# CliqueOfficial/zk-dcap-verifier

Measured on AMD Instinct MI355X. Metric: proofs/hour sgx_dcap_verifier k=19 (create_proof on the GPU: commitments, lookups, grand products, NTTs, evaluate_h, evaluations, SHPLONK, host transcript; witness synthesis excluded), higher is better.
Workload: dtype u32x8 (256-bit Montgomery integers)

## Files before the change

### zk-dcap-verifier_amd/csrc/capi.hip

```cpp
#include <string.h>
#include <new>
#include <system_error>
#include "quotient.h"

namespace zk {
int ntt_set_lds_attr();
int quotient_set_lds_attr();
int domain_lagrange_to_coeff(zk_ctx* ctx, void* d_a, uint32_t k);
int domain_coeff_to_lagrange(zk_ctx* ctx, void* d_a, uint32_t k);
int domain_lagrange_to_coeff_batch(zk_ctx* ctx, void* const* cols, size_t count, uint32_t k);
int domain_coeff_to_extended_batch(zk_ctx* ctx, const void* const* coeffs, void* const* outs, size_t count, uint32_t k, uint32_t ek);
int ntt_dev_batch(zk_ctx* ctx, void* const* h_cols, const void* const* h_srcs, size_t count, uint32_t log_n, const u256& omega, const NttFuse* fuse);
int domain_coeff_to_extended(zk_ctx* ctx, const void* d_coeff, uint32_t k, uint32_t ek, void* d_out);
int domain_extended_to_coeff(zk_ctx* ctx, void* d_a, uint32_t k, uint32_t ek);
int domain_divide_by_vanishing(zk_ctx* ctx, void* d_a, uint32_t k, uint32_t ek);
int fr_vec_op(zk_ctx* ctx, int op, const void* a, const void* b, void* out, size_t n, const u256* scalar);
int permutation_product(zk_ctx* ctx, const void* const* values, const void* const* sigmas, size_t count, uint32_t k, const void* beta, const void* gamma,
                        const void* delta_start, const void* z_init, const void* blinding, uint32_t bf, void* d_z, void* h_last_z);
int lookup_product(zk_ctx* ctx, const void* cin, const void* ctab, const void* pin, const void* ptab, uint32_t k, const void* beta, const void* gamma,
                   const void* blinding, uint32_t bf, void* d_z);
int permutation_product_circuits(zk_ctx* ctx, const void* const* values, const void* const* sigmas, size_t m, size_t n_circuits, uint32_t chunk_len, uint32_t k,
                                 const void* beta, const void* gamma, const void* blinding, uint32_t bf, void* const* d_zs);
int lookup_product_batch(zk_ctx* ctx, const void* const* cols4, size_t count, uint32_t k, const void* beta, const void* gamma, const void* blinding,
                         uint32_t bf, void* const* d_zs);
int eval_polynomial_batch(zk_ctx* ctx, const void* const* polys, size_t count, size_t n, const void* points, void* out);
int kate_division(zk_ctx* ctx, const void* d_a, size_t n, const void* b_host, void* d_q);
int fr_lincomb(zk_ctx* ctx, const void* const* polys, const void* scalars, size_t count, size_t n, void* d_out);
int pk_load(zk_ctx* ctx, uint64_t prog, const void* const* fixed, const void* const* sigma, const void* l0, const void* l_last, const void* l_active,
            int form, uint64_t* handle);
int pk_release(zk_ctx* ctx, uint64_t h);
void release_pks(zk_ctx* ctx);
int evaluate_h_host(zk_ctx* ctx, uint64_t pkh, const void* const* advice, const void* const* instance, const void* const* perm_products,
                    const void* const* lk_product, const void* const* lk_input, const void* const* lk_table, const void* challenges,
                    const void* beta, const void* gamma, const void* theta, const void* y, int finish, void* out);
int lookup_permute(zk_ctx* ctx, const void* d_input, const void* d_table, uint32_t k, uint32_t blinding_factors, const void* h_blind_input,
                   const void* h_blind_table, void* d_out_input, void* d_out_table);
int lookup_permute_batch(zk_ctx* ctx, const void* const* d_inputs, const void* const* d_tables, size_t count, uint32_t k, uint32_t blinding_factors,
                         const void* h_blind_inputs, const void* h_blind_tables, void* const* d_out_inputs, void* const* d_out_tables);
int g1_decompress(zk_ctx* ctx, const void* d_bytes, size_t n, uint32_t sign_bit, void* d_out_affine, uint32_t* n_bad_host);
int g1_compress(zk_ctx* ctx, const void* d_affine, size_t n, uint32_t sign_bit, void* d_bytes);
int g1_ntt(zk_ctx* ctx, const void* d_affine_in, uint32_t log_n, const void* omega_host, const void* scale_host, void* d_affine_out);
int quotient_program_load(zk_ctx* ctx, const void* blob, size_t len, uint64_t* prog);
int quotient_program_release(zk_ctx* ctx, uint64_t prog);
int quotient_program_info(zk_ctx* ctx, uint64_t prog, uint32_t* n_instr, uint32_t* n_slots, uint32_t* n_columns);
int quotient_program_kernels(zk_ctx* ctx, uint64_t prog, uint32_t* n_kernels);
int quotient_program_opmix(zk_ctx* ctx, uint64_t prog, uint32_t part, uint32_t counts[9]);
int mock_prover_verify(zk_ctx* ctx, const zk_mock_desc* d, zk_mock_failure* out, size_t cap, uint64_t counts[3], size_t* n_written, const void* challenges = nullptr,
                       uint32_t n_challenges = 0, bool phased = false);
int mock_prover_open(zk_ctx* ctx, const zk_mock_desc* d, uint64_t* mp);
int mock_prover_check(zk_ctx* ctx, uint64_t mp, const zk_mock_witness* w, zk_mock_failure* out, size_t cap, uint64_t counts[3], size_t* n_written);
int mock_prover_info(zk_ctx* ctx, uint64_t mp, zk_mock_info* info);
int mock_prover_close(zk_ctx* ctx, uint64_t mp);
int quotient_program_split(zk_ctx* ctx, uint64_t prog, uint32_t* low_cosets, uint32_t* n_instr_high, uint32_t* n_instr_low);
int domain_coeff_to_coset_batch(zk_ctx* ctx, const void* const* coeffs, void* const* outs, size_t count, uint32_t k, uint32_t ek, uint32_t coset);
int fr_interleave(zk_ctx* ctx, const void* const* h_cosets, size_t count, size_t n, void* d_out);
int domain_cosets_to_pieces(zk_ctx* ctx, void* const* h_numer, uint32_t q, uint32_t k, uint32_t ek, void* const* h_pieces);
}
using namespace zk;

int zk::abi_exception(zk_ctx* ctx, const char* fn) noexcept {
    int code = ZK_ERR_HIP;
    char msg[sizeof ctx->err];
    try { throw; }
    catch (const zk::AbiError& e) { code = e.code; snprintf(msg, sizeof msg, "%s: %s", fn, e.what ? e.what : "internal error"); }
    catch (const std::bad_alloc&) { code = ZK_ERR_LIMIT; snprintf(msg, sizeof msg, "%s: out of host memory (std::bad_alloc)", fn); }
    catch (const std::system_error& e) { snprintf(msg, sizeof msg, "%s: %s (std::system_error %d: no thread or lock to be had)", fn, e.what(), e.code().value()); }
    catch (const std::exception& e) { snprintf(msg, sizeof msg, "%s: unexpected C++ exception: %s", fn, e.what()); }
    catch (...) { snprintf(msg, sizeof msg, "%s: unexpected C++ exception", fn); }
    if (ctx) {
        try { std::lock_guard<std::mutex> lk(ctx->mu); memcpy(ctx->err, msg, sizeof msg); }
        catch (...) { memcpy(ctx->err, msg, sizeof msg); }
    }
    return code;
}

#ifdef ZK_FAULT_INJECT
#include <atomic>
namespace {
thread_local long g_fail_alloc_in = 0;
thread_local long g_alloc_count = 0;
std::atomic<long> g_fail_alloc_any{0};
thread_local int g_fail_thread = 0;
}
#if defined(__has_feature)
#if __has_feature(address_sanitizer) || __has_feature(thread_sanitizer)
#define ZK_NO_NEW_HOOK 1
#endif
#endif
#ifndef ZK_NO_NEW_HOOK
void* operator new(size_t n) {
    g_alloc_count++;
    if (g_fail_alloc_in > 0 && --g_fail_alloc_in == 0) throw std::bad_alloc();
    if (g_fail_alloc_any.load(std::memory_order_relaxed) > 0 && g_fail_alloc_any.fetch_sub(1) == 1) throw std::bad_alloc();
    void* p = malloc(n ? n : 1);
    if (!p) throw std::bad_alloc();
    return p;
}
void* operator new[](size_t n) { return operator new(n); }
void operator delete(void* p) noexcept { free(p); }
void operator delete[](void* p) noexcept { free(p); }
void operator delete(void* p, size_t) noexcept { free(p); }
void operator delete[](void* p, size_t) noexcept { free(p); }
#endif
void zk::fault_thread_tick() { if (g_fail_thread > 0 && --g_fail_thread == 0) throw std::system_error(std::make_error_code(std::errc::resource_unavailable_try_again), "std::thread"); }
extern "C" {
int zk_test_alloc_hook_present(void) {
#ifdef ZK_NO_NEW_HOOK
    return 0;
#else
    return 1;
#endif
}
void zk_test_fail_alloc(long nth) { g_fail_alloc_in = nth; g_alloc_count = 0; }
void zk_test_fail_alloc_any_thread(long nth) { g_fail_alloc_any.store(nth); }
long zk_test_alloc_count(void) { return g_alloc_count; }
void zk_test_fail_thread(int nth) { g_fail_thread = nth; }
#ifdef ZK_EMU
long zk_test_live_device_allocs(void) { return emu_live_device_allocs.load(); }
#endif
}
#endif

void zk_internal_plonk_ctx_destroyed(zk_ctx* ctx);
int zk_internal_fail(zk_ctx* ctx, int code, const char* msg) { return ctx ? ctx->fail(code, "%s", msg) : code; }
#define LOCK std::lock_guard<std::mutex> lk__(ctx->mu)
#define NEED_CTX if (!ctx) return ZK_ERR_ARG

extern "C" {

const char* zk_version(void) ZK_ABI_TRY {
#ifdef ZK_EMU
    return "zkmi355 0.1 (EMULATED kernels - test build, not the product)";
#else
    return "zkmi355 0.1 gfx950";
#endif
} ZK_ABI_CATCH_VALUE(nullptr, "zkmi355: internal error")

uint32_t zk_abi_version(void) ZK_ABI_TRY { return ZK_ABI_VERSION; } ZK_ABI_CATCH_VALUE(nullptr, 0u)
uint32_t zk_abi_struct_size(const char* name) ZK_ABI_TRY {
    if (!name) return 0;
    if (!strcmp(name, "zk_quotient_args")) return (uint32_t)sizeof(zk_quotient_args);
    if (!strcmp(name, "zk_plonk_pk_desc")) return (uint32_t)sizeof(zk_plonk_pk_desc);
    if (!strcmp(name, "zk_plonk_pk_host")) return (uint32_t)sizeof(zk_plonk_pk_host);
    if (!strcmp(name, "zk_mock_desc")) return (uint32_t)sizeof(zk_mock_desc);
    if (!strcmp(name, "zk_mock_failure")) return (uint32_t)sizeof(zk_mock_failure);
    if (!strcmp(name, "zk_plonk_phases")) return (uint32_t)sizeof(zk_plonk_phases);
    if (!strcmp(name, "zk_plonk_keygen_desc")) return (uint32_t)sizeof(zk_plonk_keygen_desc);
    if (!strcmp(name, "zk_mock_witness")) return (uint32_t)sizeof(zk_mock_witness);
    if (!strcmp(name, "zk_mock_info")) return (uint32_t)sizeof(zk_mock_info);
    return 0;
} ZK_ABI_CATCH_VALUE(nullptr, 0u)

int zk_ctx_create(int device_id, zk_ctx** out) ZK_ABI_TRY {
    if (!out) return ZK_ERR_ARG;
    *out = nullptr;
#ifndef ZK_EMU
    int ndev = 0;
    if (hipGetDeviceCount(&ndev) != hipSuccess || ndev <= 0 || device_id < 0 || device_id >= ndev) return ZK_ERR_NODEV;
    if (hipSetDevice(device_id) != hipSuccess) return ZK_ERR_NODEV;
#endif
    std::unique_ptr<zk_ctx> ctx(new zk_ctx());
    ctx->device = device_id;
    if (hipStreamCreateWithFlags(&ctx->stream, hipStreamNonBlocking) != hipSuccess) return ZK_ERR_HIP;
    msm_set_lds_attr();
    ntt_set_lds_attr();
    quotient_set_lds_attr();
    *out = ctx.release();
    return ZK_OK;
} ZK_ABI_CATCH(nullptr)

}
zk_ctx* zk_internal_helper_ctx(zk_ctx* ctx) {
    if (!ctx) return nullptr;
    zk_ctx* h;
    {
        LOCK;
        h = ctx->helper;
    }
    if (!h) {
        zk_ctx* made = nullptr;
        if (zk_ctx_create(ctx->device, &made) != ZK_OK) return nullptr;
#ifndef ZK_EMU
        {
            int lane_prio;
            { LOCK; lane_prio = ctx->tune.prover_lane_priority; }
            int least = 0, greatest = 0;
            hipStream_t s = nullptr;
            if (lane_prio && hipDeviceGetStreamPriorityRange(&least, &greatest) == hipSuccess && least != greatest &&
                hipStreamCreateWithPriority(&s, hipStreamNonBlocking, lane_prio == 1 ? least : greatest) == hipSuccess) {
                (void)hipStreamDestroy(made->stream);
                made->stream = s;
            }
        }
#endif
        {
            LOCK;
            if (!ctx->helper) { ctx->helper = made; made = nullptr; }
            h = ctx->helper;
        }
        if (made) zk_ctx_destroy(made);
    }
    zk::Tune t;
    bool timing;
    {
        LOCK;
        t = ctx->tune; timing = ctx->timing;
    }
    std::lock_guard<std::mutex> lk(h->mu);
    h->tune = t;
    h->timing = timing;
    return h;
}
static void release_workspaces(zk_ctx* ctx) {
    zk::DevBuf* bufs[] = {&ctx->ws_scalars, &ctx->ws_sorted, &ctx->ws_mid, &ctx->ws_small, &ctx->ws_sub0, &ctx->ws_sub1, &ctx->ws_cls0,
                          &ctx->ws_cls1, &ctx->ws_tmp, &ctx->ws_ntt, &ctx->ws_ntt_in, &ctx->ws_pts, &ctx->ws_runs, &ctx->ws_quot, &ctx->ws_quot_state};
    for (auto* b : bufs) b->release();
}
void zk_internal_trim_helper(zk_ctx* ctx) {
    if (!ctx) return;
    zk_ctx* h;
    { LOCK; h = ctx->helper; }
    if (!h) return;
    std::lock_guard<std::mutex> lk(h->mu);
    (void)hipSetDevice(h->device);
    (void)hipStreamSynchronize(h->stream);
    release_workspaces(h);
    release_twiddles(h);
}
extern "C" {
void zk_ctx_destroy(zk_ctx* ctx) ZK_ABI_TRY {
    if (!ctx) return;
    zk_ctx* helper;
    { LOCK; helper = ctx->helper; ctx->helper = nullptr; }
    if (helper) zk_ctx_destroy(helper);
    zk_internal_plonk_ctx_destroyed(ctx);
    (void)zk_plonk_trim(ctx);
    {
        LOCK;
        (void)hipSetDevice(ctx->device);
        (void)hipStreamSynchronize(ctx->stream);
        ctx->bases.clear();
        drop_pending_timers(ctx);
        release_twiddles(ctx);
        release_pks(ctx);
        release_mock_sessions(ctx);
        release_programs(ctx);
        release_gtab(ctx);
        release_workspaces(ctx);
        (void)hipStreamDestroy(ctx->stream);
    }
    delete ctx;
} ZK_ABI_CATCH_VOID(ctx)

const char* zk_last_error(zk_ctx* ctx) ZK_ABI_TRY { return ctx ? ctx->err : "null context"; } ZK_ABI_CATCH_VALUE(ctx, "zkmi355: internal error")

static int* tune_slot(zk_ctx* ctx, const char* key) {
    zk::Tune& t = ctx->tune;
    struct { const char* k; int* v; } tab[] = {
        {"msm_c", &t.msm_c}, {"msm_sort_wgs", &t.msm_sort_wgs}, {"msm_sort_threads", &t.msm_sort_threads}, {"msm_sort_batch_wgs", &t.msm_sort_batch_wgs}, {"msm_bsort_threads", &t.msm_bsort_threads}, {"msm_bsort_chunk", &t.msm_bsort_chunk}, {"msm_wide_bins_log", &t.msm_wide_bins_log}, {"msm_part_threads", &t.msm_part_threads}, {"msm_part_pairs", &t.msm_part_pairs}, {"msm_two_level_sort", &t.msm_two_level_sort},
        {"msm_target_threads", &t.msm_target_threads}, {"msm_min_chunk", &t.msm_min_chunk}, {"msm_max_chunk", &t.msm_max_chunk},
        {"msm_max_chunk_wide", &t.msm_max_chunk_wide}, {"msm_merge_fanin", &t.msm_merge_fanin}, {"msm_tree_fanin", &t.msm_tree_fanin}, {"msm_block", &t.msm_block}, {"msm_runs", &t.msm_runs}, {"prover_side_lane", &t.prover_side_lane}, {"prover_lane_priority", &t.prover_lane_priority},
        {"ntt_tile_log", &t.ntt_tile_log}, {"ntt_threads", &t.ntt_threads}, {"ntt_max_radix_log", &t.ntt_max_radix_log}, {"ntt_plan", &t.ntt_plan}, {"ntt_full_twiddle_max_log", &t.ntt_full_twiddle_max_log}, {"ntt_coset_table", &t.ntt_coset_table}, {"ntt_col_major", &t.ntt_col_major},
        {"vec_block", &t.vec_block}, {"quot_threads", &t.quot_threads},
        {"ntt_quarter_input", &t.ntt_quarter_input}, {"ntt_fuse_scale", &t.ntt_fuse_scale}, {"quot_piece_cosets", &t.quot_piece_cosets}, {"quot_factor_horner", &t.quot_factor_horner}, {"quot_degree_split", &t.quot_degree_split}, {"quot_group_factors", &t.quot_group_factors}, {"ntt_ws_limit_mb", &t.ntt_ws_limit_mb}, 
        {"quot_jit", &t.quot_jit}, {"quot_jit_group", &t.quot_jit_group}, {"quot_jit_waves", &t.quot_jit_waves}, {"quot_remat_ops", &t.quot_remat_ops}, {"quot_remat_distance", &t.quot_remat_distance}, {"keygen_wgs", &t.keygen_wgs}, {"mock_edge_wgs", &t.mock_edge_wgs}};
    for (auto& e : tab) if (!strcmp(e.k, key)) return e.v;
    return nullptr;
}
int zk_tune_set(zk_ctx* ctx, const char* key, int value) ZK_ABI_TRY {
    NEED_CTX; LOCK;
    int* s = key ? tune_slot(ctx, key) : nullptr;
    if (!s) return ctx->fail(ZK_ERR_ARG, "zk_tune_set: unknown key '%s'", key ? key : "(null)");
    if (value < 0) return ctx->fail(ZK_ERR_ARG, "zk_tune_set: negative value");
    *s = value;
    return ZK_OK;
} ZK_ABI_CATCH(ctx)
int zk_tune_get(zk_ctx* ctx, const char* key, int* value) ZK_ABI_TRY {
    NEED_CTX; LOCK;
    int* s = key ? tune_slot(ctx, key) : nullptr;
    if (!s || !value) return ctx->fail(ZK_ERR_ARG, "zk_tune_get: unknown key '%s'", key ? key : "(null)");
    *value = *s;
    return ZK_OK;
} ZK_ABI_CATCH(ctx)
int zk_timing_enable(zk_ctx* ctx, int on) ZK_ABI_TRY {
    NEED_CTX;
    zk_ctx* helper;
    { LOCK; helper = ctx->helper; }
    if (helper) (void)zk_timing_enable(helper, on);
    LOCK;
    resolve_pending_timers(ctx);
    if (on) ctx->last_ms.clear();
    ctx->timing = on != 0;
    return ZK_OK;
} ZK_ABI_CATCH(ctx)
double zk_timing_get(zk_ctx* ctx, const char* label) ZK_ABI_TRY {
    if (!ctx || !label) return -1.0;
    zk_ctx* helper;
    { LOCK; helper = ctx->helper; }
    const double side = helper ? zk_timing_get(helper, label) : -1.0;
    LOCK;
    resolve_pending_timers(ctx);
    auto it = ctx->last_ms.find(label);
    if (it == ctx->last_ms.end()) return side;
    return it->second + (side > 0 ? side : 0.0);
} ZK_ABI_CATCH_VALUE(ctx, -1.0)

#define ENTER NEED_CTX; LOCK; ZK_HIP(hipSetDevice(ctx->device))

int zk_dev_alloc(zk_ctx* ctx, size_t bytes, void** dptr) ZK_ABI_TRY { ENTER; if (!dptr) return ctx->fail(ZK_ERR_ARG, "null"); ZK_HIP(hipMalloc(dptr, bytes ? bytes : 32)); return ZK_OK; } ZK_ABI_CATCH(ctx)
int zk_dev_free(zk_ctx* ctx, void* dptr) ZK_ABI_TRY { ENTER; ZK_HIP(hipFree(dptr)); return ZK_OK; } ZK_ABI_CATCH(ctx)
int zk_dev_upload(zk_ctx* ctx, void* dptr, const void* host, size_t bytes) ZK_ABI_TRY {
    ENTER; if ((!dptr || !host) && bytes) return ctx->fail(ZK_ERR_ARG, "zk_dev_upload: null");
    ZK_HIP(hipMemcpyAsync(dptr, host, bytes, hipMemcpyHostToDevice, ctx->stream)); ZK_HIP(hipStreamSynchronize(ctx->stream)); return ZK_OK;
} ZK_ABI_CATCH(ctx)
int zk_dev_download(zk_ctx* ctx, void* host, const void* dptr, size_t bytes) ZK_ABI_TRY {
    ENTER; if ((!dptr || !host) && bytes) return ctx->fail(ZK_ERR_ARG, "zk_dev_download: null");
    ZK_HIP(hipMemcpyAsync(host, dptr, bytes, hipMemcpyDeviceToHost, ctx->stream)); ZK_HIP(hipStreamSynchronize(ctx->stream)); return ZK_OK;
} ZK_ABI_CATCH(ctx)
int zk_dev_copy(zk_ctx* ctx, void* dst, const void* src, size_t bytes) ZK_ABI_TRY {
    ENTER; if ((!dst || !src) && bytes) return ctx->fail(ZK_ERR_ARG, "zk_dev_copy: null");
    ZK_HIP(hipMemcpyAsync(dst, src, bytes, hipMemcpyDeviceToDevice, ctx->stream)); ZK_HIP(hipStreamSynchronize(ctx->stream)); return ZK_OK;
} ZK_ABI_CATCH(ctx)
int zk_dev_zero(zk_ctx* ctx, void* dptr, size_t bytes) ZK_ABI_TRY {
    ENTER; if (!dptr && bytes) return ctx->fail(ZK_ERR_ARG, "zk_dev_zero: null");
    ZK_HIP(hipMemsetAsync(dptr, 0, bytes, ctx->stream)); return ZK_OK;
} ZK_ABI_CATCH(ctx)
int zk_dev_sync(zk_ctx* ctx) ZK_ABI_TRY { ENTER; ZK_HIP(hipStreamSynchronize(ctx->stream)); return ZK_OK; } ZK_ABI_CATCH(ctx)
int zk_host_alloc(zk_ctx* ctx, size_t bytes, void** hptr) ZK_ABI_TRY {
    ENTER; if (!hptr) return ctx->fail(ZK_ERR_ARG, "zk_host_alloc: null");
    ZK_HIP(hipHostMalloc(hptr, bytes ? bytes : 32, 0)); return ZK_OK;
} ZK_ABI_CATCH(ctx)
int zk_host_free(zk_ctx* ctx, void* hptr) ZK_ABI_TRY { ENTER; ZK_HIP(hipHostFree(hptr)); return ZK_OK; } ZK_ABI_CATCH(ctx)
int zk_dev_upload_batch(zk_ctx* ctx, void* const* dptrs, const void* const* hosts, size_t count, size_t bytes_each) ZK_ABI_TRY {
    ENTER; if ((!dptrs || !hosts) && count) return ctx->fail(ZK_ERR_ARG, "zk_dev_upload_batch: null");
    for (size_t i = 0; i < count; i++) {
        if (!dptrs[i] || !hosts[i]) return ctx->fail(ZK_ERR_ARG, "zk_dev_upload_batch: null column %zu", i);
        ZK_HIP(hipMemcpyAsync(dptrs[i], hosts[i], bytes_each, hipMemcpyHostToDevice, ctx->stream));
    }
    ZK_HIP(hipStreamSynchronize(ctx->stream)); return ZK_OK;
} ZK_ABI_CATCH(ctx)

int zk_bases_register(zk_ctx* ctx, const void* p, size_t n, uint64_t* h) ZK_ABI_TRY { ENTER; return msm_register(ctx, p, n, false, h); } ZK_ABI_CATCH(ctx)
int zk_bases_register_dev(zk_ctx* ctx, const void* p, size_t n, uint64_t* h) ZK_ABI_TRY { ENTER; return msm_register(ctx, p, n, true, h); } ZK_ABI_CATCH(ctx)
int zk_bases_release(zk_ctx* ctx, uint64_t h) ZK_ABI_TRY { ENTER; return msm_release(ctx, h); } ZK_ABI_CATCH(ctx)
int zk_bases_enable_runs(zk_ctx* ctx, uint64_t h) ZK_ABI_TRY { ENTER; return msm_enable_runs(ctx, h); } ZK_ABI_CATCH(ctx)
int zk_bases_share(zk_ctx* ctx, zk_ctx* owner, uint64_t owner_handle, uint64_t* h) ZK_ABI_TRY {
    if (!ctx || !owner || !h) return ZK_ERR_ARG;
    zk::BaseTable bt;
    {
        std::lock_guard<std::mutex> lk(owner->mu);
        auto it = owner->bases.find(owner_handle);
        if (it == owner->bases.end()) return ZK_ERR_ARG;
        bt = it->second;
    }
    LOCK;
    if (owner->device != ctx->device) return ctx->fail(ZK_ERR_ARG, "zk_bases_share: the contexts are on different devices (%d, %d)", owner->device, ctx->device);
    return msm_share(ctx, bt, h);
} ZK_ABI_CATCH(ctx)
int zk_msm(zk_ctx* ctx, uint64_t b, const void* s, size_t n, void* out) ZK_ABI_TRY { ENTER; return msm_run(ctx, b, s, n, false, out, 0); } ZK_ABI_CATCH(ctx)
int zk_msm_dev(zk_ctx* ctx, uint64_t b, const void* s, size_t n, void* out) ZK_ABI_TRY { ENTER; return msm_run(ctx, b, s, n, true, out, 0); } ZK_ABI_CATCH(ctx)
int zk_msm_batch(zk_ctx* ctx, uint64_t b, const void* const* s, size_t count, size_t n, void* out) ZK_ABI_TRY { ENTER; return msm_run_batch(ctx, b, s, count, n, false, out, 0); } ZK_ABI_CATCH(ctx)
int zk_msm_batch_dev(zk_ctx* ctx, uint64_t b, const void* const* s, size_t count, size_t n, void* out) ZK_ABI_TRY { ENTER; return msm_run_batch(ctx, b, s, count, n, true, out, 0); } ZK_ABI_CATCH(ctx)
int zk_msm_partial_dev(zk_ctx* ctx, uint64_t b, const void* s, size_t n, void* out) ZK_ABI_TRY { ENTER; return msm_run(ctx, b, s, n, true, out, 1); } ZK_ABI_CATCH(ctx)
int zk_msm_batch_partial_dev(zk_ctx* ctx, uint64_t b, const void* const* s, size_t count, size_t n, void* out) ZK_ABI_TRY { ENTER; return msm_run_batch(ctx, b, s, count, n, true, out, 1); } ZK_ABI_CATCH(ctx)
int zk_g1_sum_xyzz_batch(const void* xyzz, size_t parts, size_t count, void* out) ZK_ABI_TRY {
    if (!xyzz || !out) return ZK_ERR_ARG;
    for (size_t c = 0; c < count; c++) {
        std::vector<unsigned char> col(parts * 128);
        for (size_t p = 0; p < parts; p++) memcpy(&col[p * 128], (const char*)xyzz + (p * count + c) * 128, 128);
        int rc = g1_sum_xyzz_host(col.data(), parts, (char*)out + c * 96);
        if (rc) return rc;
    }
    return ZK_OK;
} ZK_ABI_CATCH(nullptr)
int zk_g1_sum_xyzz(const void* xyzz, size_t count, void* out) ZK_ABI_TRY { if (!xyzz || !out) return ZK_ERR_ARG; return g1_sum_xyzz_host(xyzz, count, out); } ZK_ABI_CATCH(nullptr)
int zk_g1_fixed_base_mul_dev(zk_ctx* ctx, const void* s, size_t n, void* out) ZK_ABI_TRY { ENTER; return g1_fixed_base_mul(ctx, s, n, out); } ZK_ABI_CATCH(ctx)

int zk_g1_ntt_dev(zk_ctx* ctx, const void* in, uint32_t log_n, const void* omega, const void* scale, void* out) ZK_ABI_TRY { ENTER; return g1_ntt(ctx, in, log_n, omega, scale, out); } ZK_ABI_CATCH(ctx)

int zk_g1_decompress_dev(zk_ctx* ctx, const void* bytes_dev, size_t n, uint32_t sign_bit, void* out_affine_dev, uint32_t* n_invalid) ZK_ABI_TRY { ENTER; return g1_decompress(ctx, bytes_dev, n, sign_bit, out_affine_dev, n_invalid); } ZK_ABI_CATCH(ctx)
int zk_g1_compress_dev(zk_ctx* ctx, const void* affine_dev, size_t n, uint32_t sign_bit, void* bytes_dev) ZK_ABI_TRY { ENTER; return g1_compress(ctx, affine_dev, n, sign_bit, bytes_dev); } ZK_ABI_CATCH(ctx)

static int with_host_buffer(zk_ctx* ctx, void* host_in_out, size_t in_bytes, size_t buf_bytes, size_t out_bytes, void** dbuf) {
    ZK_HIP(ctx->ws_ntt_in.ensure(buf_bytes));
    *dbuf = ctx->ws_ntt_in.p;
    (void)out_bytes;
    ZK_HIP(hipMemcpyAsync(*dbuf, host_in_out, in_bytes, hipMemcpyHostToDevice, ctx->stream));
    return ZK_OK;
}
static int finish_host(zk_ctx* ctx, void* host, const void* dbuf, size_t bytes) {
    ZK_HIP(hipMemcpyAsync(host, dbuf, bytes, hipMemcpyDeviceToHost, ctx->stream));
    ZK_HIP(hipStreamSynchronize(ctx->stream));
    return ZK_OK;
}
static u256 load_host_fr(const void* p) { u256 o; memcpy(&o, p, 32); return o; }

int zk_ntt_dev(zk_ctx* ctx, void* a, uint32_t log_n, const void* omega) ZK_ABI_TRY {
    ENTER; if (!omega) return ctx->fail(ZK_ERR_ARG, "zk_ntt: null omega");
    int rc = ntt_dev(ctx, a, log_n, load_host_fr(omega), nullptr); if (rc) return rc;
    ZK_HIP(hipStreamSynchronize(ctx->stream)); return ZK_OK;
} ZK_ABI_CATCH(ctx)
int zk_ntt(zk_ctx* ctx, void* a, uint32_t log_n, const void* omega) ZK_ABI_TRY {
    ENTER; if (!omega || !a) return ctx->fail(ZK_ERR_ARG, "zk_ntt: null pointer");
    if (log_n > 27) return ctx->fail(ZK_ERR_LIMIT, "zk_ntt: log_n = %u > 27", log_n);
    void* d; size_t bytes = (size_t)32 << log_n;
    int rc = with_host_buffer(ctx, a, bytes, bytes, bytes, &d); if (rc) return rc;
    rc = ntt_dev(ctx, d, log_n, load_host_fr(omega), nullptr); if (rc) return rc;
    return finish_host(ctx, a, d, bytes);
} ZK_ABI_CATCH(ctx)
int zk_ntt_batch_dev(zk_ctx* ctx, void* const* cols, size_t count, uint32_t log_n, const void* omega) ZK_ABI_TRY {
    ENTER; if (!omega) return ctx->fail(ZK_ERR_ARG, "zk_ntt_batch_dev: null omega");
    int rc = ntt_dev_batch(ctx, cols, nullptr, count, log_n, load_host_fr(omega), nullptr); if (rc) return rc;
    ZK_HIP(hipStreamSynchronize(ctx->stream)); return ZK_OK;
} ZK_ABI_CATCH(ctx)
int zk_lagrange_to_coeff_batch_dev(zk_ctx* ctx, void* const* cols, size_t count, uint32_t k) ZK_ABI_TRY {
    ENTER; int rc = domain_lagrange_to_coeff_batch(ctx, cols, count, k); if (rc) return rc; ZK_HIP(hipStreamSynchronize(ctx->stream)); return ZK_OK;
} ZK_ABI_CATCH(ctx)
int zk_coeff_to_extended_batch_dev(zk_ctx* ctx, const void* const* coeffs, void* const* outs, size_t count, uint32_t k, uint32_t ek) ZK_ABI_TRY {
    ENTER; int rc = domain_coeff_to_extended_batch(ctx, coeffs, outs, count, k, ek); if (rc) return rc; ZK_HIP(hipStreamSynchronize(ctx->stream)); return ZK_OK;
} ZK_ABI_CATCH(ctx)
int zk_coeff_to_coset_batch_dev(zk_ctx* ctx, const void* const* coeffs, void* const* outs, size_t count, uint32_t k, uint32_t ek, uint32_t coset) ZK_ABI_TRY {
    ENTER; int rc = domain_coeff_to_coset_batch(ctx, coeffs, outs, count, k, ek, coset); if (rc) return rc; ZK_HIP(hipStreamSynchronize(ctx->stream)); return ZK_OK;
} ZK_ABI_CATCH(ctx)
int zk_fr_interleave_dev(zk_ctx* ctx, const void* const* cosets, size_t count, size_t n, void* out) ZK_ABI_TRY { ENTER; return fr_interleave(ctx, cosets, count, n, out); } ZK_ABI_CATCH(ctx)
int zk_cosets_to_pieces_dev(zk_ctx* ctx, void* const* numer, uint32_t pieces, uint32_t k, uint32_t ek, void* const* out) ZK_ABI_TRY { ENTER; return domain_cosets_to_pieces(ctx, numer, pieces, k, ek, out); } ZK_ABI_CATCH(ctx)
int zk_lagrange_to_coeff_dev(zk_ctx* ctx, void* a, uint32_t k) ZK_ABI_TRY { ENTER; int rc = domain_lagrange_to_coeff(ctx, a, k); if (rc) return rc; ZK_HIP(hipStreamSynchronize(ctx->stream)); return ZK_OK; } ZK_ABI_CATCH(ctx)
int zk_coeff_to_lagrange_dev(zk_ctx* ctx, void* a, uint32_t k) ZK_ABI_TRY { ENTER; int rc = domain_coeff_to_lagrange(ctx, a, k); if (rc) return rc; ZK_HIP(hipStreamSynchronize(ctx->stream)); return ZK_OK; } ZK_ABI_CATCH(ctx)
int zk_coeff_to_extended_dev(zk_ctx* ctx, const void* c, uint32_t k, uint32_t ek, void* out) ZK_ABI_TRY { ENTER; int rc = domain_coeff_to_extended(ctx, c, k, ek, out); if (rc) return rc; ZK_HIP(hipStreamSynchronize(ctx->stream)); return ZK_OK; } ZK_ABI_CATCH(ctx)
int zk_extended_to_coeff_dev(zk_ctx* ctx, void* a, uint32_t k, uint32_t ek) ZK_ABI_TRY { ENTER; int rc = domain_extended_to_coeff(ctx, a, k, ek); if (rc) return rc; ZK_HIP(hipStreamSynchronize(ctx->stream)); return ZK_OK; } ZK_ABI_CATCH(ctx)
int zk_divide_by_vanishing_poly_dev(zk_ctx* ctx, void* a, uint32_t k, uint32_t ek) ZK_ABI_TRY { ENTER; return domain_divide_by_vanishing(ctx, a, k, ek); } ZK_ABI_CATCH(ctx)

int zk_lagrange_to_coeff(zk_ctx* ctx, void* a, uint32_t k) ZK_ABI_TRY {
    ENTER; if (!a || k > 27) return ctx->fail(ZK_ERR_ARG, "zk_lagrange_to_coeff: bad argument");
    void* d; size_t bytes = (size_t)32 << k;
    int rc = with_host_buffer(ctx, a, bytes, bytes, bytes, &d); if (rc) return rc;
    rc = domain_lagrange_to_coeff(ctx, d, k); if (rc) return rc;
    return finish_host(ctx, a, d, bytes);
} ZK_ABI_CATCH(ctx)
int zk_coeff_to_extended(zk_ctx* ctx, const void* c, uint32_t k, uint32_t ek, void* out) ZK_ABI_TRY {
    ENTER; if (!c || !out || k > ek || ek > 27) return ctx->fail(ZK_ERR_ARG, "zk_coeff_to_extended: bad argument");
    size_t inb = (size_t)32 << k, outb = (size_t)32 << ek;
    ZK_HIP(ctx->ws_ntt_in.ensure(inb + outb));
    void* din = ctx->ws_ntt_in.p; void* dout = (char*)din + inb;
    ZK_HIP(hipMemcpyAsync(din, c, inb, hipMemcpyHostToDevice, ctx->stream));
    int rc = domain_coeff_to_extended(ctx, din, k, ek, dout); if (rc) return rc;
    return finish_host(ctx, out, dout, outb);
} ZK_ABI_CATCH(ctx)
int zk_extended_to_coeff(zk_ctx* ctx, void* a, uint32_t k, uint32_t ek) ZK_ABI_TRY {
    ENTER; if (!a || k > ek || ek > 27) return ctx->fail(ZK_ERR_ARG, "zk_extended_to_coeff: bad argument");
    void* d; size_t bytes = (size_t)32 << ek;
    int rc = with_host_buffer(ctx, a, bytes, bytes, bytes, &d); if (rc) return rc;
    rc = domain_extended_to_coeff(ctx, d, k, ek); if (rc) return rc;
    return finish_host(ctx, a, d, bytes);
} ZK_ABI_CATCH(ctx)

static int vec_sync(zk_ctx* ctx, int rc) { if (rc) return rc; ZK_HIP(hipStreamSynchronize(ctx->stream)); return ZK_OK; }
int zk_fr_mul_dev(zk_ctx* ctx, const void* a, const void* b, void* o, size_t n) ZK_ABI_TRY { ENTER; return vec_sync(ctx, fr_vec_op(ctx, 0, a, b, o, n, nullptr)); } ZK_ABI_CATCH(ctx)
int zk_fr_add_dev(zk_ctx* ctx, const void* a, const void* b, void* o, size_t n) ZK_ABI_TRY { ENTER; return vec_sync(ctx, fr_vec_op(ctx, 1, a, b, o, n, nullptr)); } ZK_ABI_CATCH(ctx)
int zk_fr_sub_dev(zk_ctx* ctx, const void* a, const void* b, void* o, size_t n) ZK_ABI_TRY { ENTER; return vec_sync(ctx, fr_vec_op(ctx, 2, a, b, o, n, nullptr)); } ZK_ABI_CATCH(ctx)
int zk_fr_scale_dev(zk_ctx* ctx, const void* a, const void* s, void* o, size_t n) ZK_ABI_TRY {
    ENTER; if (!s) return ctx->fail(ZK_ERR_ARG, "zk_fr_scale_dev: null scalar");
    u256 sc = load_host_fr(s); return vec_sync(ctx, fr_vec_op(ctx, 3, a, nullptr, o, n, &sc));
} ZK_ABI_CATCH(ctx)
int zk_fq_mul_dev(zk_ctx* ctx, const void* a, const void* b, void* o, size_t n) ZK_ABI_TRY { ENTER; return vec_sync(ctx, fr_vec_op(ctx, 4, a, b, o, n, nullptr)); } ZK_ABI_CATCH(ctx)

int zk_permutation_product_dev(zk_ctx* ctx, const void* const* values, const void* const* sigmas, size_t count, uint32_t k, const void* beta,
                               const void* gamma, const void* delta_start, const void* z_init, const void* blinding, uint32_t blinding_factors,
                               void* z_dev, void* last_z_out) ZK_ABI_TRY {
    ENTER; return permutation_product(ctx, values, sigmas, count, k, beta, gamma, delta_start, z_init, blinding, blinding_factors, z_dev, last_z_out);
} ZK_ABI_CATCH(ctx)
int zk_lookup_product_dev(zk_ctx* ctx, const void* cin, const void* ctab, const void* pin, const void* ptab, uint32_t k, const void* beta,
                          const void* gamma, const void* blinding, uint32_t blinding_factors, void* z_dev) ZK_ABI_TRY {
    ENTER; return lookup_product(ctx, cin, ctab, pin, ptab, k, beta, gamma, blinding, blinding_factors, z_dev);
} ZK_ABI_CATCH(ctx)

int zk_permutation_product_all_dev(zk_ctx* ctx, const void* const* values, const void* const* sigmas, size_t n_columns, uint32_t chunk_len, uint32_t k,
                                   const void* beta, const void* gamma, const void* blinding, uint32_t blinding_factors, void* const* z_devs) ZK_ABI_TRY {
    ENTER; return permutation_product_circuits(ctx, values, sigmas, n_columns, 1, chunk_len, k, beta, gamma, blinding, blinding_factors, z_devs);
} ZK_ABI_CATCH(ctx)
}
int zk_internal_permutation_products(zk_ctx* ctx, const void* const* values, const void* const* sigmas, size_t n_columns, size_t n_circuits, uint32_t chunk_len, uint32_t k,
                                     const void* beta, const void* gamma, const void* blinding, uint32_t blinding_factors, void* const* z_devs) {
    ENTER; return permutation_product_circuits(ctx, values, sigmas, n_columns, n_circuits, chunk_len, k, beta, gamma, blinding, blinding_factors, z_devs);
}
extern "C" {
int zk_lookup_product_batch_dev(zk_ctx* ctx, const void* const* cols4, size_t count, uint32_t k, const void* beta, const void* gamma, const void* blinding,
                                uint32_t blinding_factors, void* const* z_devs) ZK_ABI_TRY {
    ENTER; return lookup_product_batch(ctx, cols4, count, k, beta, gamma, blinding, blinding_factors, z_devs);
} ZK_ABI_CATCH(ctx)

int zk_lookup_permute_dev(zk_ctx* ctx, const void* input, const void* table, uint32_t k, uint32_t blinding_factors, const void* blind_input,
                          const void* blind_table, void* out_input, void* out_table) ZK_ABI_TRY {
    ENTER; return lookup_permute(ctx, input, table, k, blinding_factors, blind_input, blind_table, out_input, out_table);
} ZK_ABI_CATCH(ctx)

int zk_lookup_permute_batch_dev(zk_ctx* ctx, const void* const* inputs, const void* const* tables, size_t count, uint32_t k, uint32_t blinding_factors,
                                const void* blind_inputs, const void* blind_tables, void* const* out_inputs, void* const* out_tables) ZK_ABI_TRY {
    ENTER; return lookup_permute_batch(ctx, inputs, tables, count, k, blinding_factors, blind_inputs, blind_tables, out_inputs, out_tables);
} ZK_ABI_CATCH(ctx)

int zk_eval_polynomial_batch_dev(zk_ctx* ctx, const void* const* polys, size_t count, size_t n, const void* points, void* out) ZK_ABI_TRY {
    ENTER; return eval_polynomial_batch(ctx, polys, count, n, points, out);
} ZK_ABI_CATCH(ctx)
int zk_kate_division_dev(zk_ctx* ctx, const void* a_dev, size_t n, const void* b, void* q_dev) ZK_ABI_TRY { ENTER; return kate_division(ctx, a_dev, n, b, q_dev); } ZK_ABI_CATCH(ctx)
int zk_fr_lincomb_dev(zk_ctx* ctx, const void* const* polys_dev, const void* scalars, size_t count, size_t n, void* out_dev) ZK_ABI_TRY { ENTER; return fr_lincomb(ctx, polys_dev, scalars, count, n, out_dev); } ZK_ABI_CATCH(ctx)

int zk_quotient_program_load(zk_ctx* ctx, const void* blob, size_t len, uint64_t* prog) ZK_ABI_TRY { ENTER; return quotient_program_load(ctx, blob, len, prog); } ZK_ABI_CATCH(ctx)
int zk_quotient_program_info(zk_ctx* ctx, uint64_t prog, uint32_t* ni, uint32_t* ns, uint32_t* nc) ZK_ABI_TRY { ENTER; return quotient_program_info(ctx, prog, ni, ns, nc); } ZK_ABI_CATCH(ctx)
int zk_quotient_program_kernels(zk_ctx* ctx, uint64_t prog, uint32_t* n_kernels) ZK_ABI_TRY { ENTER; return quotient_program_kernels(ctx, prog, n_kernels); } ZK_ABI_CATCH(ctx)
int zk_quotient_program_opmix(zk_ctx* ctx, uint64_t prog, uint32_t counts[9]) ZK_ABI_TRY { ENTER; return quotient_program_opmix(ctx, prog, 0, counts); } ZK_ABI_CATCH(ctx)
int zk_quotient_program_part_opmix(zk_ctx* ctx, uint64_t prog, uint32_t part, uint32_t counts[9]) ZK_ABI_TRY { ENTER; return quotient_program_opmix(ctx, prog, part, counts); } ZK_ABI_CATCH(ctx)
int zk_quotient_program_release(zk_ctx* ctx, uint64_t prog) ZK_ABI_TRY { ENTER; return quotient_program_release(ctx, prog); } ZK_ABI_CATCH(ctx)
int zk_quotient_program_share(zk_ctx* ctx, zk_ctx* owner, uint64_t owner_prog, uint64_t* prog) ZK_ABI_TRY {
    if (!ctx || !owner || !prog) return ZK_ERR_ARG;
    return quotient_program_share(ctx, owner, owner_prog, prog);
} ZK_ABI_CATCH(ctx)
#define ARGS_SIZE(fn) do { if (!args) return ctx->fail(ZK_ERR_ARG, fn ": null args"); \
        if (args->struct_size != sizeof(zk_quotient_args)) return ctx->fail(ZK_ERR_ARG, fn ": zk_quotient_args.struct_size %u, expected %zu (ABI version %u)", args->struct_size, sizeof(zk_quotient_args), ZK_ABI_VERSION); } while (0)
int zk_mock_prover_verify(zk_ctx* ctx, const zk_mock_desc* desc, zk_mock_failure* out, size_t cap, uint64_t counts[3], size_t* n_written) ZK_ABI_TRY {
    ENTER; return mock_prover_verify(ctx, desc, out, cap, counts, n_written);
} ZK_ABI_CATCH(ctx)
int zk_mock_prover_verify_phased(zk_ctx* ctx, const zk_mock_desc* desc, const void* challenges, uint32_t n_challenges, zk_mock_failure* out, size_t cap,
                                 uint64_t counts[3], size_t* n_written) ZK_ABI_TRY {
    ENTER;
    if (n_challenges && !challenges) return ctx->fail(ZK_ERR_ARG, "zk_mock_prover_verify_phased: %u challenges and a null array", n_challenges);
    if (n_challenges > ZK_MAX_CHALLENGES) return ctx->fail(ZK_ERR_LIMIT, "zk_mock_prover_verify_phased: %u challenges, the quotient interpreter's constant bank is sized for %u", n_challenges, ZK_MAX_CHALLENGES);
    return mock_prover_verify(ctx, desc, out, cap, counts, n_written, challenges, n_challenges, true);
} ZK_ABI_CATCH(ctx)
int zk_mock_prover_open(zk_ctx* ctx, const zk_mock_desc* desc, uint64_t* mp) ZK_ABI_TRY { ENTER; return mock_prover_open(ctx, desc, mp); } ZK_ABI_CATCH(ctx)
int zk_mock_prover_check(zk_ctx* ctx, uint64_t mp, const zk_mock_witness* w, zk_mock_failure* out, size_t cap, uint64_t counts[3], size_t* n_written) ZK_ABI_TRY {
    ENTER; return mock_prover_check(ctx, mp, w, out, cap, counts, n_written);
} ZK_ABI_CATCH(ctx)
int zk_mock_prover_info(zk_ctx* ctx, uint64_t mp, zk_mock_info* info) ZK_ABI_TRY { ENTER; return mock_prover_info(ctx, mp, info); } ZK_ABI_CATCH(ctx)
int zk_mock_prover_close(zk_ctx* ctx, uint64_t mp) ZK_ABI_TRY { ENTER; return mock_prover_close(ctx, mp); } ZK_ABI_CATCH(ctx)
int zk_quotient_run_dev(zk_ctx* ctx, uint64_t prog, const zk_quotient_args* args) ZK_ABI_TRY { ENTER; ARGS_SIZE("zk_quotient_run_dev"); return quotient_run(ctx, prog, args, QuotRoute{}); } ZK_ABI_CATCH(ctx)
int zk_quotient_run_coset_dev(zk_ctx* ctx, uint64_t prog, const zk_quotient_args* args, uint32_t coset) ZK_ABI_TRY {
    ENTER;
    ARGS_SIZE("zk_quotient_run_coset_dev");
    if (coset >= (1u << 16)) return ctx->fail(ZK_ERR_ARG, "zk_quotient_run_coset_dev: coset %u out of range", coset);
    QuotRoute r;
    r.coset = (int)coset;
    return quotient_run(ctx, prog, args, r);
} ZK_ABI_CATCH(ctx)
int zk_quotient_run_coset_rows_dev(zk_ctx* ctx, uint64_t prog, const zk_quotient_args* args, uint32_t coset, uint64_t row_lo, uint64_t row_count) ZK_ABI_TRY {
    ENTER;
    ARGS_SIZE("zk_quotient_run_coset_rows_dev");
    if (coset >= (1u << 16)) return ctx->fail(ZK_ERR_ARG, "zk_quotient_run_coset_rows_dev: coset %u out of range", coset);
    if (!row_count) return ctx->fail(ZK_ERR_ARG, "zk_quotient_run_coset_rows_dev: row_count = 0");
    QuotRoute r;
    r.coset = (int)coset; r.row_lo = row_lo; r.row_count = row_count;
    return quotient_run(ctx, prog, args, r);
} ZK_ABI_CATCH(ctx)
int zk_quotient_program_split(zk_ctx* ctx, uint64_t prog, uint32_t* low_cosets, uint32_t* n_instr_high, uint32_t* n_instr_low) ZK_ABI_TRY { ENTER; return quotient_program_split(ctx, prog, low_cosets, n_instr_high, n_instr_low); } ZK_ABI_CATCH(ctx)
int zk_quotient_run_high_dev(zk_ctx* ctx, uint64_t prog, const zk_quotient_args* args) ZK_ABI_TRY {
    ENTER; ARGS_SIZE("zk_quotient_run_high_dev");
    QuotRoute r;
    r.part = 1;
    return quotient_run(ctx, prog, args, r);
} ZK_ABI_CATCH(ctx)
int zk_quotient_run_low_dev(zk_ctx* ctx, uint64_t prog, const zk_quotient_args* args, uint32_t low_cosets) ZK_ABI_TRY {
    ENTER; ARGS_SIZE("zk_quotient_run_low_dev");
    if (!low_cosets) return ctx->fail(ZK_ERR_ARG, "zk_quotient_run_low_dev: low_cosets = 0");
    QuotRoute r;
    r.part = 2; r.low_cosets = low_cosets;
    return quotient_run(ctx, prog, args, r);
} ZK_ABI_CATCH(ctx)
int zk_quotient_run_coset_part_dev(zk_ctx* ctx, uint64_t prog, const zk_quotient_args* args, uint32_t coset, uint32_t part) ZK_ABI_TRY {
    ENTER; ARGS_SIZE("zk_quotient_run_coset_part_dev");
    if (coset >= (1u << 16) || part < 1 || part > 2) return ctx->fail(ZK_ERR_ARG, "zk_quotient_run_coset_part_dev: coset %u / part %u out of range", coset, part);
    QuotRoute r;
    r.coset = (int)coset; r.part = (int)part;
    return quotient_run(ctx, prog, args, r);
} ZK_ABI_CATCH(ctx)
int zk_quotient_run_acc_dev(zk_ctx* ctx, uint64_t prog, const zk_quotient_args* args, uint32_t coset, uint32_t part) ZK_ABI_TRY {
    ENTER; ARGS_SIZE("zk_quotient_run_acc_dev");
    if ((coset != UINT32_MAX && coset >= (1u << 16)) || part > 2) return ctx->fail(ZK_ERR_ARG, "zk_quotient_run_acc_dev: coset %u / part %u out of range", coset, part);
    QuotRoute r;
    r.coset = coset == UINT32_MAX ? -1 : (int)coset; r.part = (int)part; r.accumulate = true;
    if (coset == UINT32_MAX && part == 2) {
        int rc = quotient_program_split(ctx, prog, &r.low_cosets, nullptr, nullptr);
        if (rc) return rc;
        if (!r.low_cosets) return ctx->fail(ZK_ERR_ARG, "zk_quotient_run_acc_dev: program %llu has no degree split (zk_quotient_program_split)", (unsigned long long)prog);
    }
    return quotient_run(ctx, prog, args, r);
} ZK_ABI_CATCH(ctx)

int zk_pk_load(zk_ctx* ctx, uint64_t prog, const void* const* fixed, const void* const* sigma, const void* l0, const void* l_last, const void* l_active,
               int form, uint64_t* pk) ZK_ABI_TRY { ENTER; return pk_load(ctx, prog, fixed, sigma, l0, l_last, l_active, form, pk); } ZK_ABI_CATCH(ctx)
int zk_pk_release(zk_ctx* ctx, uint64_t pk) ZK_ABI_TRY { ENTER; return pk_release(ctx, pk); } ZK_ABI_CATCH(ctx)
int zk_evaluate_h(zk_ctx* ctx, uint64_t pk, const void* const* advice, const void* const* instance, const void* const* perm_products,
                  const void* const* lookup_product, const void* const* lookup_input, const void* const* lookup_table, const void* challenges,
                  const void* beta, const void* gamma, const void* theta, const void* y, int finish, void* out) ZK_ABI_TRY {
    ENTER; return evaluate_h_host(ctx, pk, advice, instance, perm_products, lookup_product, lookup_input, lookup_table, challenges, beta, gamma, theta, y, finish, out);
} ZK_ABI_CATCH(ctx)

}
```

### zk-dcap-verifier_amd/csrc/ctx.h

```cpp
#pragma once
#include <stdarg.h>
#include <string.h>
#include <stdio.h>
#include <list>
#include <map>
#include <memory>
#include <mutex>
#include <string>
#include <vector>
#include "ec.cuh"
#include "../../include/zkmi355.h"
#include "abi_guard.h"

namespace zk {

struct Tune {
    int msm_c = 0;
    int msm_sort_wgs = 256;
    int msm_sort_threads = 1024;
    int msm_bsort_threads = 1024;
    int msm_bsort_chunk = 8192;
    int msm_part_threads = 1024, msm_part_pairs = 16384;
    int msm_wide_bins_log = 9;
    int msm_two_level_sort = 0;
    int msm_sort_batch_wgs = 2048;
    int msm_target_threads = 1 << 19;
    int msm_min_chunk = 16;
    int msm_max_chunk = 48;
    int msm_max_chunk_wide = 128;
    int msm_merge_fanin = 8;
    int msm_tree_fanin = 2;
    int msm_block = 128;
    int prover_lane_priority = 1;
    int prover_side_lane = 1;
    int msm_runs = 1;
    int ntt_tile_log = 10;
    int ntt_threads = 256;
    int ntt_max_radix_log = 8;
    int ntt_plan = 0;
    int ntt_col_major = 1;
    int ntt_coset_table = 1;
    int ntt_full_twiddle_max_log = 24;
    int ntt_ws_limit_mb = 24576;
    int ntt_fuse_scale = 1;
    int ntt_quarter_input = 1;
    int vec_block = 256;
    int quot_threads = 128;
    int quot_piece_cosets = 1;
    int quot_degree_split = 1;
    int quot_group_factors = 1;
    int quot_factor_horner = 1;
    int quot_remat_ops = 4;
    int quot_remat_distance = 24;
    int quot_jit = 0;
    int quot_jit_waves = 0;
    int keygen_wgs = 2048;
    int mock_edge_wgs = 2048;
    int quot_jit_group = 200;
};

struct DevBuf {
    void* p = nullptr;
    size_t cap = 0;
    hipError_t ensure(size_t bytes) {
        if (bytes <= cap) return hipSuccess;
        if (p) (void)hipFree(p);
        p = nullptr; cap = 0;
        size_t want = bytes + bytes / 8 + 4096;
        hipError_t e = hipMalloc(&p, want);
        if (e == hipSuccess) cap = want;
        return e;
    }
    void release() { if (p) (void)hipFree(p); p = nullptr; cap = 0; }
};

struct DevTmp {
    void* p = nullptr;
    DevTmp() = default;
    DevTmp(const DevTmp&) = delete;
    DevTmp& operator=(const DevTmp&) = delete;
    ~DevTmp() { if (p) (void)hipFree(p); }
    void* release() { void* q = p; p = nullptr; return q; }
    void reset() { if (p) (void)hipFree(p); p = nullptr; }
};

struct TableMem {
    void* p = nullptr;
    int device = 0;
    ~TableMem() { if (p) { (void)hipSetDevice(device); (void)hipFree(p); } }
};
struct BaseTable {
    void* d_table = nullptr;
    size_t n = 0;
    int c = 0, W = 0;
    std::shared_ptr<TableMem> mem;
    void* d_runs_table = nullptr;
    std::shared_ptr<TableMem> runs_mem;
};

struct TwiddleSet {
    uint32_t log_n = 0;
    u256 omega;
    void* d_lo = nullptr;
    void* d_hi = nullptr;
    uint32_t lo_bits = 0;
    void* d_stage[3] = {nullptr, nullptr, nullptr};
    void* d_stage_sh[3] = {nullptr, nullptr, nullptr};
    void* d_stage29[3] = {nullptr, nullptr, nullptr};
    void* d_full[3] = {nullptr, nullptr, nullptr};
    uint32_t radix_log[3] = {0, 0, 0};
    int passes = 0;
    bool scale_fused = false;
    u256 fused_scale;
    uint64_t stamp = 0;
};

struct QuotProgram;
struct MockSession;

}

struct zk_ctx {
    int device = 0;
    std::mutex mu;
    char err[640] = {0};
    hipStream_t stream = nullptr;
    zk::Tune tune;
    uint64_t next_handle = 1;
    std::map<uint64_t, zk::BaseTable> bases;
    std::list<zk::TwiddleSet> twiddles;
    uint64_t twiddle_clock = 0;
    std::map<uint64_t, void*> coset_tables;
    std::map<uint64_t, std::shared_ptr<zk::QuotProgram>> programs;
    std::map<uint64_t, std::shared_ptr<zk::MockSession>> mock_sessions;
    std::map<uint64_t, std::vector<uint32_t>> lookup_tie_hint;
    zk::DevBuf ws_scalars, ws_sorted, ws_mid, ws_small, ws_sub0, ws_sub1, ws_cls0, ws_cls1, ws_tmp, ws_ntt, ws_ntt_in, ws_pts, ws_runs, ws_quot, ws_quot_state;
    bool timing = false;
    std::map<std::string, double> last_ms;
    struct PendingTimer { const char* label; hipEvent_t a, b; };
    std::vector<PendingTimer> pending_timers;
    zk_ctx* helper = nullptr;

    int fail(int code, const char* fmt, ...) {
        char buf[sizeof err];
        va_list ap;
        va_start(ap, fmt);
        vsnprintf(buf, sizeof buf, fmt, ap);
        va_end(ap);
        memcpy(err, buf, sizeof err);
        return code;
    }
};

#define ZK_HIP(call)                                                                          \
    do {                                                                                      \
        hipError_t e__ = (call);                                                              \
        if (e__ != hipSuccess)                                                                \
            return ctx->fail(ZK_ERR_HIP, "%s failed: %s (%s:%d)", #call, hipGetErrorString(e__), __FILE__, __LINE__); \
    } while (0)
#define ZK_CHECK_LAUNCH() ZK_HIP(hipGetLastError())

namespace zk {
inline void resolve_pending_timers(zk_ctx* ctx);
struct EvTimer {
    zk_ctx* ctx; const char* label; hipEvent_t a = nullptr, b = nullptr; bool on;
    EvTimer(zk_ctx* c, const char* l) : ctx(c), label(l), on(c->timing) {
        if (on) { (void)hipEventCreate(&a); (void)hipEventCreate(&b); (void)hipEventRecord(a, ctx->stream); }
    }
    void stop() { if (on) (void)hipEventRecord(b, ctx->stream); }
    void resolve() {
        if (!on) return;
        (void)hipEventSynchronize(b);
        float ms = 0; (void)hipEventElapsedTime(&ms, a, b);
        on = false;
        (void)hipEventDestroy(a); (void)hipEventDestroy(b);
        ctx->last_ms[label] += ms; ctx->last_ms[std::string(label) + "#n"] += 1.0;
    }
    void defer() {
        if (!on) return;
        if (ctx->pending_timers.size() >= 4096) resolve_pending_timers(ctx);
        ctx->pending_timers.push_back({label, a, b});
        on = false;
    }
    ~EvTimer() { if (on) { (void)hipEventDestroy(a); (void)hipEventDestroy(b); } }
    EvTimer(const EvTimer&) = delete;
    EvTimer& operator=(const EvTimer&) = delete;
};
inline void resolve_pending_timers(zk_ctx* ctx) {
    std::vector<zk_ctx::PendingTimer> list;
    list.swap(ctx->pending_timers);
    struct Drop { std::vector<zk_ctx::PendingTimer>& l; ~Drop() { for (auto& t : l) { (void)hipEventDestroy(t.a); (void)hipEventDestroy(t.b); } } } drop{list};
    for (auto& t : list) {
        (void)hipEventSynchronize(t.b);
        float ms = 0; (void)hipEventElapsedTime(&ms, t.a, t.b);
        ctx->last_ms[t.label] += ms; ctx->last_ms[std::string(t.label) + "#n"] += 1.0;
    }
}
inline void drop_pending_timers(zk_ctx* ctx) {
    for (auto& t : ctx->pending_timers) { (void)hipEventDestroy(t.a); (void)hipEventDestroy(t.b); }
    ctx->pending_timers.clear();
}

int msm_register(zk_ctx* ctx, const void* pts, size_t n, bool on_device, uint64_t* handle);
int msm_release(zk_ctx* ctx, uint64_t handle);
int msm_share(zk_ctx* dst, const BaseTable& bt, uint64_t* handle);
int msm_enable_runs(zk_ctx* ctx, uint64_t handle);
int msm_run(zk_ctx* ctx, uint64_t handle, const void* scalars, size_t n, bool on_device, void* out, int partial);
int msm_run_batch(zk_ctx* ctx, uint64_t handle, const void* const* scalars, size_t nb, size_t n, bool on_device, void* out, int partial);
int g1_sum_xyzz_host(const void* xyzz, size_t count, void* out_jac);
int g1_fixed_base_mul(zk_ctx* ctx, const void* d_scalars, size_t n, void* d_out_affine);
void release_gtab(zk_ctx* ctx);
int msm_set_lds_attr();
struct NttFuse {
    const void* src = nullptr;
    uint32_t n_valid = 0;
    int pre_zeta = 0;
    int post_scale = 0;
    u256 scale;
    int post_zeta_inv = 0;
    const void* cs_lo = nullptr; const void* cs_hi = nullptr; uint32_t cs_lo_bits = 0, cs_stride = 0, cs_log = 0;
    const void* pre_full = nullptr;
};
int ntt_dev(zk_ctx* ctx, void* d_a, uint32_t log_n, const u256& omega, const NttFuse* fuse);
void release_twiddles(zk_ctx* ctx);
void release_programs(zk_ctx* ctx);
void release_mock_sessions(zk_ctx* ctx);
int quotient_program_share(zk_ctx* ctx, zk_ctx* owner, uint64_t owner_prog, uint64_t* prog);
}
```

### zk-dcap-verifier_amd/csrc/lookupperm.hip

```cpp
#include "ctx.h"
#include <vector>

namespace zk {

constexpr uint32_t FS_T = 256, FS_E = 16, FS_TILE = FS_T * FS_E, FS_PAD = 258;

ZK_HD uint32_t fs_digit(uint2 k, uint32_t pass) { return ((pass < 4 ? k.x : k.y) >> (8 * (pass & 3))) & 255u; }

constexpr uint32_t XS_T = 256, XS_E = 8, XS_TILE = XS_T * XS_E;

ZK_HD int lp_cmp(const u256& a, const u256& b) {
    for (int i = 7; i >= 0; i--) {
        if (a.v[i] < b.v[i]) return -1;
        if (a.v[i] > b.v[i]) return 1;
    }
    return 0;
}
static uint32_t lp_scan_threads(uint32_t m) {
    uint32_t t = 64;
    while (t < 1024 && t * 8 < m) t <<= 1;
    return t;
}

struct LpbArgs {
    const void* const* cols;
    void* const* outs;
    const void* const* scols;
    const uint32_t* tabcol;
    uint32_t u, n, nb, S, C, nwg, nxs;
    void* canon; uint2* key_a; uint2* key_b; uint32_t* idx_a; uint32_t* idx_b;
    uint32_t* flags; uint32_t* ranks; uint32_t* leftover; uint32_t* ghist; uint32_t* xsums; uint32_t* scal;
    uint32_t* cscal;
    const uint32_t* shifts;
    const void* blind;
};
ZK_KERNEL void lpb_canon_kernel(LpbArgs a) {
    __shared__ uint32_t lor[8];
    const uint32_t s = blockIdx.y, i = blockIdx.x * blockDim.x + threadIdx.x;
    if (threadIdx.x < 8) lor[threadIdx.x] = 0;
    __syncthreads();
    if (i < a.u) {
        const u256 c = Fr::from_mont(load_u256(a.scols[s], i));
        store_u256(a.canon, (size_t)s * a.u + i, c);
#pragma unroll
        for (int w = 0; w < 8; w++) if (c.v[w] & ~lor[w]) atomicOr(&lor[w], c.v[w]);
    }
    __syncthreads();
    if (threadIdx.x < 8 && lor[threadIdx.x]) atomicOr(&a.cscal[s * 16 + threadIdx.x], lor[threadIdx.x]);
}
ZK_KERNEL void lpb_keys_kernel(LpbArgs a) {
    const uint32_t s = blockIdx.y, i = blockIdx.x * blockDim.x + threadIdx.x;
    if (i >= a.u) return;
    const uint32_t shift = a.shifts[s];
    const uint32_t* w = reinterpret_cast<const uint32_t*>(a.canon) + ((size_t)s * a.u + i) * 8;
    const uint32_t ws = shift >> 5, bs = shift & 31;
    uint32_t x[3];
#pragma unroll
    for (int j = 0; j < 3; j++) x[j] = ws + j < 8 ? w[ws + j] : 0u;
    uint2 k;
    k.x = bs ? (x[0] >> bs) | (x[1] << (32 - bs)) : x[0];
    k.y = bs ? (x[1] >> bs) | (x[2] << (32 - bs)) : x[1];
    a.key_a[(size_t)s * a.u + i] = k;
    a.idx_a[(size_t)s * a.u + i] = i;
}
ZK_KERNEL void lpb_hist_kernel(const uint2* keys, uint32_t u, uint32_t pass, uint32_t* ghist, uint32_t nwg) {
    __shared__ uint32_t lh[256];
    const uint32_t s = blockIdx.y, tid = threadIdx.x, base = blockIdx.x * FS_TILE;
    keys += (size_t)s * u;
    lh[tid] = 0;
    __syncthreads();
    for (uint32_t e = 0; e < FS_E; e++) {
        const uint32_t i = base + e * FS_T + tid;
        bool live = i < u;
        const uint32_t d = live ? fs_digit(keys[i], pass) : 0u;
#ifndef ZK_EMU
#pragma unroll
        for (int round = 0; round < 2; round++) {
            if (live) {
                const uint32_t lead = (uint32_t)__builtin_amdgcn_readfirstlane((int)d);
                const bool same = d == lead;
                const unsigned long long m = __ballot(same);
                if (same) {
                    if ((__lane_id() & 63u) == (uint32_t)__builtin_ctzll(m)) atomicAdd(&lh[lead], (uint32_t)__builtin_popcountll(m));
                    live = false;
                }
            }
        }
#endif
        if (live) atomicAdd(&lh[d], 1u);
    }
    __syncthreads();
    ghist[((size_t)s * nwg + blockIdx.x) * 256 + tid] = lh[tid];
}
ZK_KERNEL void lpb_offsets_kernel(uint32_t* ghist, uint32_t nwg) {
    __shared__ uint32_t scan[256];
    const uint32_t s = blockIdx.x, tid = threadIdx.x;
    uint32_t* h = ghist + (size_t)s * nwg * 256;
    uint32_t total = 0;
    for (uint32_t w = 0; w < nwg; w++) total += h[(size_t)w * 256 + tid];
    scan[tid] = total;
    __syncthreads();
    for (uint32_t d = 1; d < 256; d <<= 1) {
        const uint32_t add = tid >= d ? scan[tid - d] : 0;
        __syncthreads();
        scan[tid] += add;
        __syncthreads();
    }
    uint32_t run = scan[tid] - total;
    for (uint32_t w = 0; w < nwg; w++) {
        const uint32_t c = h[(size_t)w * 256 + tid];
        h[(size_t)w * 256 + tid] = run;
        run += c;
    }
}
ZK_KERNEL void lpb_scatter_kernel(const uint2* keys_in, const uint32_t* idx_in, uint2* keys_out, uint32_t* idx_out, uint32_t u, uint32_t pass,
                                  const uint32_t* gbase_all, uint32_t nwg) {
    __shared__ __attribute__((aligned(16))) uint16_t cnt[FS_T * FS_PAD];
    __shared__ uint32_t gbase[256];
    const uint32_t s = blockIdx.y, tid = threadIdx.x, wg = blockIdx.x, base = wg * FS_TILE;
    keys_in += (size_t)s * u; idx_in += (size_t)s * u; keys_out += (size_t)s * u; idx_out += (size_t)s * u;
    {
        uint4* c4 = reinterpret_cast<uint4*>(cnt);
        constexpr uint32_t n4 = FS_T * FS_PAD * 2 / 16;
        for (uint32_t q = tid; q < n4; q += FS_T) c4[q] = make_uint4(0, 0, 0, 0);
    }
    gbase[tid] = gbase_all[((size_t)s * nwg + wg) * 256 + tid];
    __syncthreads();
    uint2 k[FS_E];
    uint32_t v[FS_E];
    uint16_t rl[FS_E];
    const uint32_t lo = base + tid * FS_E;
#pragma unroll
    for (uint32_t e = 0; e < FS_E; e++) {
        const uint32_t i = lo + e;
        if (i < u) {
            k[e] = keys_in[i]; v[e] = idx_in[i];
            rl[e] = cnt[tid * FS_PAD + fs_digit(k[e], pass)]++;
        }
    }
    __syncthreads();
    {
        uint32_t run = 0;
        for (uint32_t t = 0; t < FS_T; t++) {
            const uint32_t c = cnt[t * FS_PAD + tid];
            cnt[t * FS_PAD + tid] = (uint16_t)run;
            run += c;
        }
    }
    __syncthreads();
#pragma unroll
    for (uint32_t e = 0; e < FS_E; e++) {
        const uint32_t i = lo + e;
        if (i < u) {
            const uint32_t d = fs_digit(k[e], pass);
            const uint32_t pos = gbase[d] + cnt[tid * FS_PAD + d] + rl[e];
            keys_out[pos] = k[e];
            idx_out[pos] = v[e];
        }
    }
}
ZK_KERNEL void lpb_check_kernel(LpbArgs a, const uint32_t* idx_sorted) {
    const uint32_t s = blockIdx.y, i = blockIdx.x * blockDim.x + threadIdx.x;
    if (i == 0 || i >= a.u || a.shifts[s] == 0) return;
    const uint32_t* canon = reinterpret_cast<const uint32_t*>(a.canon) + (size_t)s * a.u * 8;
    const uint32_t* idx = idx_sorted + (size_t)s * a.u;
    const uint32_t* x = canon + (size_t)idx[i - 1] * 8;
    const uint32_t* y = canon + (size_t)idx[i] * 8;
    for (int w = 7; w >= 0; w--) {
        if (x[w] < y[w]) return;
        if (x[w] > y[w]) { atomicAdd(&a.cscal[s * 16 + 8], 1u); return; }
    }
}
ZK_KERNEL void lpb_tiemask_kernel(LpbArgs a, const uint32_t* idx_sorted) {
    __shared__ uint32_t lor[8];
    const uint32_t s = blockIdx.y, i = blockIdx.x * blockDim.x + threadIdx.x;
    if (a.cscal[s * 16 + 8] == 0) return;
    if (threadIdx.x < 8) lor[threadIdx.x] = 0;
    __syncthreads();
    if (i > 0 && i < a.u) {
        const uint32_t shift = a.shifts[s];
        const uint32_t* canon = reinterpret_cast<const uint32_t*>(a.canon) + (size_t)s * a.u * 8;
        const uint32_t* idx = idx_sorted + (size_t)s * a.u;
        const uint32_t* x = canon + (size_t)idx[i - 1] * 8;
        const uint32_t* y = canon + (size_t)idx[i] * 8;
        uint32_t d[8], above = 0;
#pragma unroll
        for (int w = 0; w < 8; w++) {
            d[w] = x[w] ^ y[w];
            const uint32_t lo_bit = (uint32_t)w * 32;
            uint32_t in_window = lo_bit + 32 <= shift ? 0u : (lo_bit >= shift ? 0xffffffffu : (0xffffffffu << (shift - lo_bit)));
            above |= d[w] & in_window;
        }
        if (above == 0) {
#pragma unroll
            for (int w = 0; w < 8; w++) if (d[w] & ~lor[w]) atomicOr(&lor[w], d[w]);
        }
    }
    __syncthreads();
    if (threadIdx.x < 8 && lor[threadIdx.x]) atomicOr(&a.cscal[s * 16 + threadIdx.x], lor[threadIdx.x]);
}
ZK_KERNEL void lpb_rekey_kernel(LpbArgs a, const uint32_t* fcols, const uint32_t* fshift, const uint32_t* idx_in, uint2* key_out, uint32_t* idx_out) {
    const uint32_t f = blockIdx.y, i = blockIdx.x * blockDim.x + threadIdx.x;
    if (i >= a.u) return;
    const uint32_t c = fcols[f], shift = fshift[f];
    const uint32_t r = idx_in ? idx_in[(size_t)f * a.u + i] : i;
    const uint32_t* w = reinterpret_cast<const uint32_t*>(a.canon) + ((size_t)c * a.u + r) * 8;
    const uint32_t ws = shift >> 5, bs = shift & 31;
    uint32_t x[3];
#pragma unroll
    for (int j = 0; j < 3; j++) x[j] = ws + j < 8 ? w[ws + j] : 0u;
    uint2 k;
    k.x = bs ? (x[0] >> bs) | (x[1] << (32 - bs)) : x[0];
    k.y = bs ? (x[1] >> bs) | (x[2] << (32 - bs)) : x[1];
    key_out[(size_t)f * a.u + i] = k;
    idx_out[(size_t)f * a.u + i] = r;
}
ZK_KERNEL void lpb_mark_kernel(LpbArgs a, const uint32_t* idx_sorted) {
    const uint32_t l = blockIdx.y, i = blockIdx.x * blockDim.x + threadIdx.x, u = a.u;
    if (i >= u) return;
    const uint32_t tc = a.tabcol[l];
    const void* in_canon = (const char*)a.canon + (size_t)l * u * 32;
    const void* tab_canon = (const char*)a.canon + (size_t)tc * u * 32;
    const uint32_t* in_idx = idx_sorted + (size_t)l * u;
    const uint32_t* tab_idx = idx_sorted + (size_t)tc * u;
    uint32_t* repeated = a.flags + (size_t)(2 * l) * u;
    uint32_t* unconsumed = a.flags + (size_t)(2 * l + 1) * u;
    const u256 v = load_u256(in_canon, in_idx[i]);
    const bool first = i == 0 || lp_cmp(v, load_u256(in_canon, in_idx[i - 1])) != 0;
    repeated[i] = first ? 0u : 1u;
    if (!first) return;
    uint32_t lo = 0, hi = u;
    while (lo < hi) {
        const uint32_t mid = (lo + hi) >> 1;
        if (lp_cmp(load_u256(tab_canon, tab_idx[mid]), v) < 0) lo = mid + 1; else hi = mid;
    }
    if (lo >= u || lp_cmp(load_u256(tab_canon, tab_idx[lo]), v) != 0) { atomicAdd(&a.scal[l * 16 + 1], 1u); return; }
    unconsumed[lo] = 0;
}
ZK_KERNEL void lpb_fill_unconsumed_kernel(LpbArgs a) {
    const uint32_t l = blockIdx.y, i = blockIdx.x * blockDim.x + threadIdx.x;
    if (i < a.u) a.flags[(size_t)(2 * l + 1) * a.u + i] = 1u;
}
ZK_KERNEL void lpb_tile_sum_kernel(LpbArgs a) {
    __shared__ uint32_t part[XS_T];
    const uint32_t s = blockIdx.y, tid = threadIdx.x, base = blockIdx.x * XS_TILE;
    const uint32_t* v = a.ranks + (size_t)s * a.u;
    uint32_t sum = 0;
    for (uint32_t e = 0; e < XS_E; e++) { const uint32_t i = base + e * XS_T + tid; if (i < a.u) sum += v[i]; }
    part[tid] = sum;
    __syncthreads();
    for (uint32_t d = XS_T >> 1; d > 0; d >>= 1) { if (tid < d) part[tid] += part[tid + d]; __syncthreads(); }
    if (tid == 0) a.xsums[(size_t)s * a.nxs + blockIdx.x] = part[0];
}
ZK_KERNEL void lpb_sum_scan_kernel(LpbArgs a) {
    __shared__ uint32_t part[1024];
    const uint32_t s = blockIdx.x, T = blockDim.x, tid = threadIdx.x, m = a.nxs - 1;
    uint32_t* v = a.xsums + (size_t)s * a.nxs;
    const uint32_t per = (m + T - 1) / T;
    const uint32_t lo = tid * per < m ? tid * per : m, hi = lo + per < m ? lo + per : m;
    uint32_t sum = 0;
    for (uint32_t i = lo; i < hi; i++) sum += v[i];
    part[tid] = sum;
    __syncthreads();
    for (uint32_t d = 1; d < T; d <<= 1) {
        const uint32_t add = tid >= d ? part[tid - d] : 0;
        __syncthreads();
        part[tid] += add;
        __syncthreads();
    }
    uint32_t run = part[tid] - sum;
    for (uint32_t i = lo; i < hi; i++) { const uint32_t x = v[i]; v[i] = run; run += x; }
    if (tid == T - 1) a.scal[(s >> 1) * 16 + 2 + (s & 1)] = part[T - 1];
}
ZK_KERNEL void lpb_apply_kernel(LpbArgs a) {
    __shared__ uint32_t part[XS_T];
    const uint32_t s = blockIdx.y, tid = threadIdx.x, lo = blockIdx.x * XS_TILE + tid * XS_E, m = a.u;
    uint32_t* v = a.ranks + (size_t)s * a.u;
    uint32_t x[XS_E], sum = 0;
#pragma unroll
    for (uint32_t e = 0; e < XS_E; e++) { x[e] = lo + e < m ? v[lo + e] : 0u; sum += x[e]; }
    part[tid] = sum;
    __syncthreads();
    for (uint32_t d = 1; d < XS_T; d <<= 1) {
        const uint32_t add = tid >= d ? part[tid - d] : 0;
        __syncthreads();
        part[tid] += add;
        __syncthreads();
    }
    uint32_t run = a.xsums[(size_t)s * a.nxs + blockIdx.x] + part[tid] - sum;
#pragma unroll
    for (uint32_t e = 0; e < XS_E; e++) { if (lo + e < m) v[lo + e] = run; run += x[e]; }
}
ZK_KERNEL void lpb_compact_kernel(LpbArgs a) {
    const uint32_t l = blockIdx.y, t = blockIdx.x * blockDim.x + threadIdx.x;
    if (t < a.u && a.flags[(size_t)(2 * l + 1) * a.u + t]) a.leftover[(size_t)l * a.u + a.ranks[(size_t)(2 * l + 1) * a.u + t]] = t;
}
ZK_KERNEL void lpb_assemble_kernel(LpbArgs a, const uint32_t* idx_sorted) {
    const uint32_t l = blockIdx.y, i = blockIdx.x * blockDim.x + threadIdx.x, u = a.u;
    if (i >= a.n) return;
    void* out_in = a.outs[2 * l];
    void* out_tab = a.outs[2 * l + 1];
    if (i >= u) {
        store_u256(out_in, i, load_u256(a.blind, (size_t)(2 * l) * a.nb + (i - u)));
        store_u256(out_tab, i, load_u256(a.blind, (size_t)(2 * l + 1) * a.nb + (i - u)));
        return;
    }
    const uint32_t* in_idx = idx_sorted + (size_t)l * u;
    const uint32_t* tab_idx = idx_sorted + (size_t)a.tabcol[l] * u;
    const u256 v = load_u256(a.cols[2 * l], in_idx[i]);
    store_u256(out_in, i, v);
    if (!a.flags[(size_t)(2 * l) * u + i]) store_u256(out_tab, i, v);
    else {
        const uint32_t n_rep = a.scal[l * 16 + 2];
        store_u256(out_tab, i, load_u256(a.cols[2 * l + 1], tab_idx[a.leftover[(size_t)l * u + (n_rep - 1 - a.ranks[(size_t)(2 * l) * u + i])]]));
    }
}

int lookup_permute_batch(zk_ctx* ctx, const void* const* d_inputs, const void* const* d_tables, size_t count, uint32_t k, uint32_t blinding_factors,
                         const void* h_blind_inputs, const void* h_blind_tables, void* const* d_out_inputs, void* const* d_out_tables) {
    if (count == 0) return ZK_OK;
    if (!d_inputs || !d_tables || !d_out_inputs || !d_out_tables || !h_blind_inputs || !h_blind_tables)
        return ctx->fail(ZK_ERR_ARG, "zk_lookup_permute_batch_dev: null argument");
    if (k < 1 || k > 26 || count > 4096) return ctx->fail(ZK_ERR_ARG, "zk_lookup_permute_batch_dev: k = %u / count = %zu out of range", k, count);
    const uint32_t n = 1u << k, nb = blinding_factors + 1;
    if (nb >= n) return ctx->fail(ZK_ERR_ARG, "zk_lookup_permute_batch_dev: blinding_factors too large");
    for (size_t l = 0; l < count; l++)
        if (!d_inputs[l] || !d_tables[l] || !d_out_inputs[l] || !d_out_tables[l]) return ctx->fail(ZK_ERR_ARG, "zk_lookup_permute_batch_dev: null column %zu", l);
    const uint32_t u = n - nb, S = 2 * (uint32_t)count;
    std::vector<const void*> scols(d_inputs, d_inputs + count);
    std::vector<uint32_t> tabcol(count);
    for (size_t l = 0; l < count; l++) {
        size_t c = count;
        while (c < scols.size() && scols[c] != d_tables[l]) c++;
        if (c == scols.size()) scols.push_back(d_tables[l]);
        tabcol[l] = (uint32_t)c;
    }
    const uint32_t C = (uint32_t)scols.size();
    const uint32_t nwg = (u + FS_TILE - 1) / FS_TILE, nxs = (u + XS_TILE - 1) / XS_TILE + 1;
    size_t off = 0;
    auto take = [&](size_t bytes) { size_t o = off; off += (bytes + 255) & ~(size_t)255; return o; };
    const size_t o_canon = take((size_t)C * u * 32), o_blind = take((size_t)S * nb * 32), o_ka = take((size_t)C * u * 8), o_kb = take((size_t)C * u * 8),
                 o_ia = take((size_t)C * u * 4), o_ib = take((size_t)C * u * 4), o_fl = take((size_t)S * u * 4), o_rk = take((size_t)S * u * 4),
                 o_lo = take((size_t)count * u * 4), o_gh = take((size_t)C * nwg * 256 * 4), o_xs = take((size_t)S * nxs * 4), o_sc = take((size_t)count * 64),
                 o_cs = take((size_t)C * 64), o_sh = take((size_t)C * 4), o_tc = take((size_t)count * 4), o_cp = take((size_t)S * sizeof(void*)),
                 o_op = take((size_t)S * sizeof(void*)), o_sp = take((size_t)C * sizeof(void*));
    ZK_HIP(ctx->ws_tmp.ensure(off + 256));
    char* base = (char*)ctx->ws_tmp.p;
    hipStream_t st = ctx->stream;
    std::vector<const void*> cols(S);
    std::vector<void*> outs(S);
    std::vector<unsigned char> blind((size_t)S * nb * 32);
    for (size_t l = 0; l < count; l++) {
        cols[2 * l] = d_inputs[l]; cols[2 * l + 1] = d_tables[l];
        outs[2 * l] = d_out_inputs[l]; outs[2 * l + 1] = d_out_tables[l];
        memcpy(&blind[(2 * l) * (size_t)nb * 32], (const char*)h_blind_inputs + l * (size_t)nb * 32, (size_t)nb * 32);
        memcpy(&blind[(2 * l + 1) * (size_t)nb * 32], (const char*)h_blind_tables + l * (size_t)nb * 32, (size_t)nb * 32);
    }
    ZK_HIP(hipMemcpyAsync(base + o_cp, cols.data(), S * sizeof(void*), hipMemcpyHostToDevice, st));
    ZK_HIP(hipMemcpyAsync(base + o_op, outs.data(), S * sizeof(void*), hipMemcpyHostToDevice, st));
    ZK_HIP(hipMemcpyAsync(base + o_sp, scols.data(), C * sizeof(void*), hipMemcpyHostToDevice, st));
    ZK_HIP(hipMemcpyAsync(base + o_tc, tabcol.data(), count * 4, hipMemcpyHostToDevice, st));
    ZK_HIP(hipMemcpyAsync(base + o_blind, blind.data(), blind.size(), hipMemcpyHostToDevice, st));
    ZK_HIP(hipMemsetAsync(base + o_sc, 0, count * 64, st));
    ZK_HIP(hipMemsetAsync(base + o_cs, 0, (size_t)C * 64, st));
    LpbArgs a;
    memset(&a, 0, sizeof a);
    a.cols = (const void* const*)(base + o_cp); a.outs = (void* const*)(base + o_op); a.scols = (const void* const*)(base + o_sp);
    a.tabcol = (const uint32_t*)(base + o_tc);
    a.u = u; a.n = n; a.nb = nb; a.S = S; a.C = C; a.nwg = nwg; a.nxs = nxs;
    a.canon = base + o_canon; a.key_a = (uint2*)(base + o_ka); a.key_b = (uint2*)(base + o_kb); a.idx_a = (uint32_t*)(base + o_ia); a.idx_b = (uint32_t*)(base + o_ib);
    a.flags = (uint32_t*)(base + o_fl); a.ranks = (uint32_t*)(base + o_rk); a.leftover = (uint32_t*)(base + o_lo); a.ghist = (uint32_t*)(base + o_gh);
    a.xsums = (uint32_t*)(base + o_xs); a.scal = (uint32_t*)(base + o_sc); a.cscal = (uint32_t*)(base + o_cs); a.shifts = (const uint32_t*)(base + o_sh);
    a.blind = base + o_blind;
    const int blk = ctx->tune.vec_block;
    const uint32_t g = (u + blk - 1) / blk;
    ZK_LAUNCH(lpb_canon_kernel, dim3(g, C), blk, 0, st, a);
    ZK_CHECK_LAUNCH();
    std::vector<uint32_t> sc((size_t)count * 16), csc((size_t)C * 16);
    ZK_HIP(hipMemcpyAsync(csc.data(), a.cscal, (size_t)C * 64, hipMemcpyDeviceToHost, st));
    ZK_HIP(hipStreamSynchronize(st));
    std::vector<uint32_t> shifts(C);
    uint32_t max_bits = 1;
    bool any_shift = false;
    for (uint32_t c = 0; c < C; c++) {
        const uint32_t* om = &csc[(size_t)c * 16];
        uint32_t nbits = 1;
        for (int wd = 7; wd >= 0; wd--)
            if (om[wd]) { uint32_t top = 31; while (!((om[wd] >> top) & 1)) top--; nbits = (uint32_t)wd * 32 + top + 1; break; }
        shifts[c] = nbits > 64 ? nbits - 64 : 0;
        any_shift |= shifts[c] != 0;
        max_bits = std::max(max_bits, std::min(nbits, 64u));
    }
    ZK_HIP(hipMemcpyAsync(base + o_sh, shifts.data(), (size_t)C * 4, hipMemcpyHostToDevice, st));
    uint32_t* sorted = a.idx_a;
    const bool use_order_check = any_shift;

    auto compact_sort = [&](const std::vector<uint32_t>& fcols, const std::vector<std::vector<uint32_t>>& stage_shift, const std::vector<uint32_t>& stage_bits) -> int {
        const uint32_t Fn = (uint32_t)fcols.size();
        if (!Fn) return ZK_OK;
        const size_t per = (size_t)Fn * u;
        size_t o2 = 0;
        auto take2 = [&](size_t bytes) { size_t o = o2; o2 += (bytes + 255) & ~(size_t)255; return o; };
        const size_t q_ka = take2(per * 8), q_kb = take2(per * 8), q_ia = take2(per * 4), q_ib = take2(per * 4), q_gh = take2((size_t)Fn * nwg * 256 * 4),
                     q_fc = take2((size_t)Fn * 4), q_fs = take2((size_t)Fn * 4 * stage_shift.size());
        ZK_HIP(ctx->ws_mid.ensure(o2 + 256));
        char* b2 = (char*)ctx->ws_mid.p;
        uint2 *rk_in = (uint2*)(b2 + q_ka), *rk_out = (uint2*)(b2 + q_kb);
        uint32_t *ri_in = (uint32_t*)(b2 + q_ia), *ri_out = (uint32_t*)(b2 + q_ib), *rgh = (uint32_t*)(b2 + q_gh);
        ZK_HIP(hipMemcpyAsync(b2 + q_fc, fcols.data(), (size_t)Fn * 4, hipMemcpyHostToDevice, st));
        for (size_t t = 0; t < stage_shift.size(); t++)
            ZK_HIP(hipMemcpyAsync(b2 + q_fs + t * Fn * 4, stage_shift[t].data(), (size_t)Fn * 4, hipMemcpyHostToDevice, st));
        const uint32_t* order = nullptr;
        for (size_t t = 0; t < stage_shift.size(); t++) {
            ZK_LAUNCH(lpb_rekey_kernel, dim3(g, Fn), blk, 0, st, a, (const uint32_t*)(b2 + q_fc), (const uint32_t*)(b2 + q_fs + t * Fn * 4), order, rk_in, ri_in);
            ZK_CHECK_LAUNCH();
            const uint32_t ps = (stage_bits[t] + 7) / 8;
            for (uint32_t p = 0; p < ps; p++) {
                ZK_LAUNCH(lpb_hist_kernel, dim3(nwg, Fn), FS_T, 0, st, (const uint2*)rk_in, u, p, rgh, nwg);
                ZK_CHECK_LAUNCH();
                ZK_LAUNCH(lpb_offsets_kernel, Fn, 256, 0, st, rgh, nwg);
                ZK_CHECK_LAUNCH();
                ZK_LAUNCH(lpb_scatter_kernel, dim3(nwg, Fn), FS_T, 0, st, (const uint2*)rk_in, (const uint32_t*)ri_in, rk_out, ri_out, u, p, (const uint32_t*)rgh, nwg);
                ZK_CHECK_LAUNCH();
                std::swap(rk_in, rk_out);
                std::swap(ri_in, ri_out);
            }
            std::swap(rk_in, rk_out);
            std::swap(ri_in, ri_out);
            order = ri_out;
        }
        for (uint32_t f = 0; f < Fn; f++)
            ZK_HIP(hipMemcpyAsync(sorted + (size_t)fcols[f] * u, order + (size_t)f * u, (size_t)u * 4, hipMemcpyDeviceToDevice, st));
        return ZK_OK;
    };
    auto low_stages = [&](const std::vector<uint32_t>& fcols, const std::vector<uint32_t>& lo_bit, const std::vector<uint32_t>& hi_bit,
                          std::vector<std::vector<uint32_t>>& stage_shift, std::vector<uint32_t>& stage_bits) {
        const uint32_t Fn = (uint32_t)fcols.size();
        uint32_t n_low = 0;
        for (uint32_t f = 0; f < Fn; f++) if (lo_bit[f] < 256) n_low = std::max(n_low, (hi_bit[f] - lo_bit[f]) / 64 + 1);
        for (uint32_t t = 0; t < n_low; t++) {
            std::vector<uint32_t> sh(Fn);
            uint32_t bits = 1;
            for (uint32_t f = 0; f < Fn; f++) {
                const uint32_t st_lo = lo_bit[f] == 256 ? 256 : lo_bit[f] + 64 * t;
                if (st_lo > hi_bit[f] || st_lo >= 256) { sh[f] = 255; continue; }
                sh[f] = st_lo;
                bits = std::max(bits, std::min(64u, hi_bit[f] - st_lo + 1));
            }
            stage_shift.push_back(sh); stage_bits.push_back(bits);
        }
        std::vector<uint32_t> sh(Fn);
        for (uint32_t f = 0; f < Fn; f++) sh[f] = shifts[fcols[f]];
        stage_shift.push_back(sh); stage_bits.push_back(max_bits);
    };
    auto tie_ranges = [&](const std::vector<uint32_t>& cols_, std::vector<uint32_t>& lo_bit, std::vector<uint32_t>& hi_bit) -> int {
        for (uint32_t c : cols_) ZK_HIP(hipMemsetAsync((char*)a.cscal + (size_t)c * 64, 0, 32, st));
        ZK_LAUNCH(lpb_tiemask_kernel, dim3(g, C), blk, 0, st, a, (const uint32_t*)sorted); ZK_CHECK_LAUNCH();
        ZK_HIP(hipMemcpyAsync(csc.data(), a.cscal, (size_t)C * 64, hipMemcpyDeviceToHost, st));
        ZK_HIP(hipStreamSynchronize(st));
        lo_bit.assign(cols_.size(), 256); hi_bit.assign(cols_.size(), 0);
        for (size_t f = 0; f < cols_.size(); f++) {
            const uint32_t* m = &csc[(size_t)cols_[f] * 16];
            for (uint32_t b = 0; b < 256; b++) if ((m[b >> 5] >> (b & 31)) & 1) { if (lo_bit[f] == 256) lo_bit[f] = b; hi_bit[f] = b; }
        }
        return ZK_OK;
    };

    const uint64_t hint_key = ((uint64_t)count << 40) ^ ((uint64_t)C << 20) ^ k;
    std::vector<uint32_t>& hint = ctx->lookup_tie_hint[hint_key];
    if (hint.size() != C) hint.assign(C, 0);
    std::vector<uint32_t> plain, hinted;
    for (uint32_t c = 0; c < C; c++) (hint[c] && shifts[c] ? hinted : plain).push_back(c);
    {
        std::vector<std::vector<uint32_t>> ss(1, std::vector<uint32_t>(plain.size()));
        for (size_t f = 0; f < plain.size(); f++) ss[0][f] = shifts[plain[f]];
        int rc = compact_sort(plain, ss, {max_bits});
        if (rc) return rc;
    }
    if (!hinted.empty()) {
        std::vector<uint32_t> lo_bit(hinted.size(), 0), hi_bit(hinted.size());
        for (size_t f = 0; f < hinted.size(); f++) hi_bit[f] = std::min(shifts[hinted[f]] - 1, hint[hinted[f]] - 1 + 16);
        std::vector<std::vector<uint32_t>> ss; std::vector<uint32_t> sb;
        low_stages(hinted, lo_bit, hi_bit, ss, sb);
        int rc = compact_sort(hinted, ss, sb);
        if (rc) return rc;
        ctx->last_ms["lookup_hinted_sorts"] += (double)hinted.size();
    }
    if (use_order_check) {
        ZK_LAUNCH(lpb_check_kernel, dim3(g, C), blk, 0, st, a, (const uint32_t*)sorted); ZK_CHECK_LAUNCH();
        ZK_HIP(hipMemcpyAsync(csc.data(), a.cscal, (size_t)C * 64, hipMemcpyDeviceToHost, st));
        ZK_HIP(hipStreamSynchronize(st));
        std::vector<uint32_t> fcols;
        for (uint32_t c = 0; c < C; c++) if (csc[(size_t)c * 16 + 8]) fcols.push_back(c);
        if (!fcols.empty()) {
            std::vector<uint32_t> lo_bit, hi_bit;
            int rc = tie_ranges(fcols, lo_bit, hi_bit);
            if (rc) return rc;
            std::vector<std::vector<uint32_t>> ss; std::vector<uint32_t> sb;
            low_stages(fcols, lo_bit, hi_bit, ss, sb);
            rc = compact_sort(fcols, ss, sb);
            if (rc) return rc;
            for (size_t f = 0; f < fcols.size(); f++) {
                hint[fcols[f]] = hi_bit[f] + 1;
                ZK_HIP(hipMemsetAsync((char*)a.cscal + (size_t)fcols[f] * 64 + 32, 0, 4, st));
            }
            ZK_LAUNCH(lpb_check_kernel, dim3(g, C), blk, 0, st, a, (const uint32_t*)sorted); ZK_CHECK_LAUNCH();
            ctx->last_ms["lookup_refined_sorts"] += (double)fcols.size();
        }
    }
    ZK_LAUNCH(lpb_fill_unconsumed_kernel, dim3(g, (uint32_t)count), blk, 0, st, a);
    ZK_CHECK_LAUNCH();
    ZK_LAUNCH(lpb_mark_kernel, dim3(g, (uint32_t)count), blk, 0, st, a, sorted);
    ZK_CHECK_LAUNCH();
    ZK_HIP(hipMemcpyAsync(a.ranks, a.flags, (size_t)S * u * 4, hipMemcpyDeviceToDevice, st));
    ZK_LAUNCH(lpb_tile_sum_kernel, dim3(nxs - 1, S), XS_T, 0, st, a);
    ZK_CHECK_LAUNCH();
    ZK_LAUNCH(lpb_sum_scan_kernel, S, lp_scan_threads(nxs - 1), 0, st, a);
    ZK_CHECK_LAUNCH();
    ZK_LAUNCH(lpb_apply_kernel, dim3(nxs - 1, S), XS_T, 0, st, a);
    ZK_CHECK_LAUNCH();
    ZK_HIP(hipMemcpyAsync(sc.data(), a.scal, count * 64, hipMemcpyDeviceToHost, st));
    ZK_HIP(hipMemcpyAsync(csc.data(), a.cscal, (size_t)C * 64, hipMemcpyDeviceToHost, st));
    ZK_HIP(hipStreamSynchronize(st));
    for (size_t l = 0; l < count; l++) {
        const uint32_t* h = &sc[l * 16];
        if (csc[l * 16 + 8] || csc[(size_t)tabcol[l] * 16 + 8])
            return ctx->fail(ZK_ERR_ARG, "zk_lookup_permute_dev: internal order violation in lookup %zu (%u input / %u table row pairs out of order after refinement)", l,
                             csc[l * 16 + 8], csc[(size_t)tabcol[l] * 16 + 8]);
        if (h[1]) return ctx->fail(ZK_ERR_ARG, "zk_lookup_permute_dev: %u input value(s) of lookup %zu are not in the table (halo2: Error::ConstraintSystemFailure)", h[1], l);
        if (h[2] != h[3]) return ctx->fail(ZK_ERR_ARG, "zk_lookup_permute_dev: internal count mismatch in lookup %zu (%u repeated rows, %u leftover table values)", l, h[2], h[3]);
    }
    ZK_LAUNCH(lpb_compact_kernel, dim3(g, (uint32_t)count), blk, 0, st, a);
    ZK_CHECK_LAUNCH();
    ZK_LAUNCH(lpb_assemble_kernel, dim3((n + blk - 1) / blk, (uint32_t)count), blk, 0, st, a, sorted);
    ZK_CHECK_LAUNCH();
    ZK_HIP(hipStreamSynchronize(st));
    ctx->last_ms["lookup_sorts"] += (double)count;
    return ZK_OK;
}
int lookup_permute(zk_ctx* ctx, const void* d_input, const void* d_table, uint32_t k, uint32_t blinding_factors, const void* h_blind_input,
                   const void* h_blind_table, void* d_out_input, void* d_out_table) {
    if (!d_input || !d_table || !d_out_input || !d_out_table || !h_blind_input || !h_blind_table)
        return ctx->fail(ZK_ERR_ARG, "zk_lookup_permute_dev: null argument");
    const void* ins[1] = {d_input}; const void* tabs[1] = {d_table};
    void* oi[1] = {d_out_input}; void* ot[1] = {d_out_table};
    return lookup_permute_batch(ctx, ins, tabs, 1, k, blinding_factors, h_blind_input, h_blind_table, oi, ot);
}

}
```

Baseline: 73400.

## Sort lookup columns on narrow adaptive key windows with local tie repair

The lookup permutation radix sort now keys each column on a window only as wide as needed for the domain size, about log2(u)+8 bits, instead of a fixed 64-bit key. Constant columns are detected and skip sorting, and per-column key widths reduce the number of radix passes. Order violations caused by ties are fixed by a new repair kernel that insertion-sorts short runs locally; long or deep runs fall back to a full 64-bit re-sort. The last pass writes indices straight into the sorted buffer instead of also copying keys. This trades fewer sort passes for extra check and repair kernels, more host synchronisation, and more complex control flow.

```diff
diff --git a/zk-dcap-verifier_amd/csrc/capi.hip b/zk-dcap-verifier_amd/csrc/capi.hip
--- a/zk-dcap-verifier_amd/csrc/capi.hip
+++ b/zk-dcap-verifier_amd/csrc/capi.hip
@@ -261,7 +261,7 @@
         {"msm_target_threads", &t.msm_target_threads}, {"msm_min_chunk", &t.msm_min_chunk}, {"msm_max_chunk", &t.msm_max_chunk},
         {"msm_max_chunk_wide", &t.msm_max_chunk_wide}, {"msm_merge_fanin", &t.msm_merge_fanin}, {"msm_tree_fanin", &t.msm_tree_fanin}, {"msm_block", &t.msm_block}, {"msm_runs", &t.msm_runs}, {"prover_side_lane", &t.prover_side_lane}, {"prover_lane_priority", &t.prover_lane_priority},
         {"ntt_tile_log", &t.ntt_tile_log}, {"ntt_threads", &t.ntt_threads}, {"ntt_max_radix_log", &t.ntt_max_radix_log}, {"ntt_plan", &t.ntt_plan}, {"ntt_full_twiddle_max_log", &t.ntt_full_twiddle_max_log}, {"ntt_coset_table", &t.ntt_coset_table}, {"ntt_col_major", &t.ntt_col_major},
-        {"vec_block", &t.vec_block}, {"quot_threads", &t.quot_threads},
+        {"vec_block", &t.vec_block}, {"quot_threads", &t.quot_threads}, {"lookup_window_bits", &t.lookup_window_bits},
         {"ntt_quarter_input", &t.ntt_quarter_input}, {"ntt_fuse_scale", &t.ntt_fuse_scale}, {"quot_piece_cosets", &t.quot_piece_cosets}, {"quot_factor_horner", &t.quot_factor_horner}, {"quot_degree_split", &t.quot_degree_split}, {"quot_group_factors", &t.quot_group_factors}, {"ntt_ws_limit_mb", &t.ntt_ws_limit_mb}, 
         {"quot_jit", &t.quot_jit}, {"quot_jit_group", &t.quot_jit_group}, {"quot_jit_waves", &t.quot_jit_waves}, {"quot_remat_ops", &t.quot_remat_ops}, {"quot_remat_distance", &t.quot_remat_distance}, {"keygen_wgs", &t.keygen_wgs}, {"mock_edge_wgs", &t.mock_edge_wgs}};
     for (auto& e : tab) if (!strcmp(e.k, key)) return e.v;
diff --git a/zk-dcap-verifier_amd/csrc/ctx.h b/zk-dcap-verifier_amd/csrc/ctx.h
--- a/zk-dcap-verifier_amd/csrc/ctx.h
+++ b/zk-dcap-verifier_amd/csrc/ctx.h
@@ -45,6 +45,7 @@
     int ntt_fuse_scale = 1;
     int ntt_quarter_input = 1;
     int vec_block = 256;
+    int lookup_window_bits = 0;
     int quot_threads = 128;
     int quot_piece_cosets = 1;
     int quot_degree_split = 1;
diff --git a/zk-dcap-verifier_amd/csrc/lookupperm.hip b/zk-dcap-verifier_amd/csrc/lookupperm.hip
--- a/zk-dcap-verifier_amd/csrc/lookupperm.hip
+++ b/zk-dcap-verifier_amd/csrc/lookupperm.hip
@@ -28,45 +28,45 @@
     const void* const* scols;
     const uint32_t* tabcol;
     uint32_t u, n, nb, S, C, nwg, nxs;
-    void* canon; uint2* key_a; uint2* key_b; uint32_t* idx_a; uint32_t* idx_b;
+    void* canon; uint32_t* sorted;
     uint32_t* flags; uint32_t* ranks; uint32_t* leftover; uint32_t* ghist; uint32_t* xsums; uint32_t* scal;
     uint32_t* cscal;
+    uint32_t* cnor;
     const uint32_t* shifts;
+    const uint32_t* shifts64;
     const void* blind;
 };
+struct LpbRow { uint32_t slot, col, src, out, shift; };
+struct LpbBufs { uint2* k[2]; uint32_t* i[2]; uint32_t* sorted; };
+constexpr uint32_t LPB_IDENTITY = 2, LPB_SORTED = 2;
+constexpr uint32_t LPB_DEEP = 1, LPB_LONG = 2;
+
 ZK_KERNEL void lpb_canon_kernel(LpbArgs a) {
-    __shared__ uint32_t lor[8];
+    __shared__ uint32_t lor[8], lnor[8];
     const uint32_t s = blockIdx.y, i = blockIdx.x * blockDim.x + threadIdx.x;
-    if (threadIdx.x < 8) lor[threadIdx.x] = 0;
+    if (threadIdx.x < 8) { lor[threadIdx.x] = 0; lnor[threadIdx.x] = 0; }
     __syncthreads();
     if (i < a.u) {
         const u256 c = Fr::from_mont(load_u256(a.scols[s], i));
         store_u256(a.canon, (size_t)s * a.u + i, c);
 #pragma unroll
-        for (int w = 0; w < 8; w++) if (c.v[w] & ~lor[w]) atomicOr(&lor[w], c.v[w]);
-    }
-    __syncthreads();
-    if (threadIdx.x < 8 && lor[threadIdx.x]) atomicOr(&a.cscal[s * 16 + threadIdx.x], lor[threadIdx.x]);
-}
-ZK_KERNEL void lpb_keys_kernel(LpbArgs a) {
-    const uint32_t s = blockIdx.y, i = blockIdx.x * blockDim.x + threadIdx.x;
-    if (i >= a.u) return;
-    const uint32_t shift = a.shifts[s];
-    const uint32_t* w = reinterpret_cast<const uint32_t*>(a.canon) + ((size_t)s * a.u + i) * 8;
-    const uint32_t ws = shift >> 5, bs = shift & 31;
-    uint32_t x[3];
-#pragma unroll
-    for (int j = 0; j < 3; j++) x[j] = ws + j < 8 ? w[ws + j] : 0u;
-    uint2 k;
-    k.x = bs ? (x[0] >> bs) | (x[1] << (32 - bs)) : x[0];
-    k.y = bs ? (x[1] >> bs) | (x[2] << (32 - bs)) : x[1];
-    a.key_a[(size_t)s * a.u + i] = k;
-    a.idx_a[(size_t)s * a.u + i] = i;
-}
-ZK_KERNEL void lpb_hist_kernel(const uint2* keys, uint32_t u, uint32_t pass, uint32_t* ghist, uint32_t nwg) {
+        for (int w = 0; w < 8; w++) {
+            if (c.v[w] & ~lor[w]) atomicOr(&lor[w], c.v[w]);
+            if (~c.v[w] & ~lnor[w]) atomicOr(&lnor[w], ~c.v[w]);
+        }
+    }
+    __syncthreads();
+    if (threadIdx.x < 8) {
+        const uint32_t o = lor[threadIdx.x], no = lnor[threadIdx.x];
+        if (o & ~*(volatile uint32_t*)&a.cscal[s * 16 + threadIdx.x]) atomicOr(&a.cscal[s * 16 + threadIdx.x], o);
+        if (no & ~*(volatile uint32_t*)&a.cnor[s * 8 + threadIdx.x]) atomicOr(&a.cnor[s * 8 + threadIdx.x], no);
+    }
+}
+ZK_KERNEL void lpb_hist_kernel(LpbBufs b, const LpbRow* rows, uint32_t u, uint32_t pass, uint32_t* ghist, uint32_t nwg) {
     __shared__ uint32_t lh[256];
     const uint32_t s = blockIdx.y, tid = threadIdx.x, base = blockIdx.x * FS_TILE;
-    keys += (size_t)s * u;
+    const LpbRow r = rows[s];
+    const uint2* keys = b.k[r.src] + (size_t)r.slot * u;
     lh[tid] = 0;
     __syncthreads();
     for (uint32_t e = 0; e < FS_E; e++) {
@@ -113,12 +113,16 @@
         run += c;
     }
 }
-ZK_KERNEL void lpb_scatter_kernel(const uint2* keys_in, const uint32_t* idx_in, uint2* keys_out, uint32_t* idx_out, uint32_t u, uint32_t pass,
-                                  const uint32_t* gbase_all, uint32_t nwg) {
+ZK_KERNEL void lpb_scatter_kernel(LpbBufs b, const LpbRow* rows, uint32_t u, uint32_t pass, const uint32_t* gbase_all, uint32_t nwg) {
     __shared__ __attribute__((aligned(16))) uint16_t cnt[FS_T * FS_PAD];
     __shared__ uint32_t gbase[256];
     const uint32_t s = blockIdx.y, tid = threadIdx.x, wg = blockIdx.x, base = wg * FS_TILE;
-    keys_in += (size_t)s * u; idx_in += (size_t)s * u; keys_out += (size_t)s * u; idx_out += (size_t)s * u;
+    const LpbRow r = rows[s];
+    const bool last = r.out == LPB_SORTED;
+    const uint2* keys_in = b.k[r.src] + (size_t)r.slot * u;
+    const uint32_t* idx_in = b.i[r.src] + (size_t)r.slot * u;
+    uint2* keys_out = last ? nullptr : b.k[r.out] + (size_t)r.slot * u;
+    uint32_t* idx_out = last ? b.sorted + (size_t)r.col * u : b.i[r.out] + (size_t)r.slot * u;
     {
         uint4* c4 = reinterpret_cast<uint4*>(cnt);
         constexpr uint32_t n4 = FS_T * FS_PAD * 2 / 16;
@@ -154,22 +158,78 @@
         if (i < u) {
             const uint32_t d = fs_digit(k[e], pass);
             const uint32_t pos = gbase[d] + cnt[tid * FS_PAD + d] + rl[e];
-            keys_out[pos] = k[e];
+            if (!last) keys_out[pos] = k[e];
             idx_out[pos] = v[e];
         }
     }
 }
-ZK_KERNEL void lpb_check_kernel(LpbArgs a, const uint32_t* idx_sorted) {
-    const uint32_t s = blockIdx.y, i = blockIdx.x * blockDim.x + threadIdx.x;
-    if (i == 0 || i >= a.u || a.shifts[s] == 0) return;
-    const uint32_t* canon = reinterpret_cast<const uint32_t*>(a.canon) + (size_t)s * a.u * 8;
-    const uint32_t* idx = idx_sorted + (size_t)s * a.u;
-    const uint32_t* x = canon + (size_t)idx[i - 1] * 8;
-    const uint32_t* y = canon + (size_t)idx[i] * 8;
+ZK_KERNEL void lpb_check_kernel(LpbArgs a, const uint32_t* idx_sorted, const uint32_t* list, uint32_t* viol) {
+    const uint32_t s = list ? list[blockIdx.y] : blockIdx.y, i = blockIdx.x * blockDim.x + threadIdx.x;
+    if (i >= a.u || a.shifts[s] == 0) return;
+    uint32_t bad = 0;
+    if (i > 0) {
+        const uint32_t* canon = reinterpret_cast<const uint32_t*>(a.canon) + (size_t)s * a.u * 8;
+        const uint32_t* idx = idx_sorted + (size_t)s * a.u;
+        const uint32_t* x = canon + (size_t)idx[i - 1] * 8;
+        const uint32_t* y = canon + (size_t)idx[i] * 8;
+        for (int w = 7; w >= 0; w--) {
+            if (x[w] < y[w]) break;
+            if (x[w] > y[w]) { bad = 1; break; }
+        }
+        if (bad) atomicAdd(&a.cscal[s * 16 + 8], 1u);
+    }
+    if (viol) viol[(size_t)s * a.u + i] = bad;
+}
+ZK_HD bool lp_same_above(const uint32_t* x, const uint32_t* y, uint32_t shift) {
+    const uint32_t ws = shift >> 5, bs = shift & 31;
+    for (uint32_t w = 7; w > ws; w--) if (x[w] != y[w]) return false;
+    return ws > 7 || ((x[ws] ^ y[ws]) >> bs) == 0;
+}
+ZK_HD int lp_cmp_words(const uint32_t* x, const uint32_t* y) {
     for (int w = 7; w >= 0; w--) {
-        if (x[w] < y[w]) return;
-        if (x[w] > y[w]) { atomicAdd(&a.cscal[s * 16 + 8], 1u); return; }
-    }
+        if (x[w] < y[w]) return -1;
+        if (x[w] > y[w]) return 1;
+    }
+    return 0;
+}
+constexpr uint32_t LPB_RUN = 16;
+ZK_KERNEL void lpb_repair_kernel(LpbArgs a, const uint32_t* list, uint32_t* idx_sorted, const uint32_t* viol_all) {
+    const uint32_t c = list[blockIdx.y], i = blockIdx.x * blockDim.x + threadIdx.x, u = a.u;
+    const uint32_t* viol = viol_all + (size_t)c * u;
+    if (i == 0 || i >= u || !viol[i]) return;
+    const uint32_t shift = a.shifts[c], shift64 = a.shifts64[c];
+    const uint32_t* canon = reinterpret_cast<const uint32_t*>(a.canon) + (size_t)c * u * 8;
+    uint32_t* idx = idx_sorted + (size_t)c * u;
+    const uint32_t* me = canon + (size_t)idx[i] * 8;
+    if (!lp_same_above(canon + (size_t)idx[i - 1] * 8, me, shift)) return;
+    uint32_t lo = i - 1;
+    while (lo > 0 && lp_same_above(canon + (size_t)idx[lo - 1] * 8, me, shift)) {
+        if (viol[lo]) return;
+        lo--;
+        if (i - lo >= LPB_RUN) { atomicOr(&a.cscal[c * 16 + 9], LPB_LONG); return; }
+    }
+    uint32_t hi = i + 1;
+    while (hi < u && lp_same_above(canon + (size_t)idx[hi] * 8, me, shift)) {
+        hi++;
+        if (hi - lo > LPB_RUN) { atomicOr(&a.cscal[c * 16 + 9], LPB_LONG); return; }
+    }
+    const uint32_t len = hi - lo;
+    uint32_t r[LPB_RUN];
+    for (uint32_t e = 0; e < len; e++) r[e] = idx[lo + e];
+    for (uint32_t e = 0; e + 1 < len; e++)
+        for (uint32_t f = e + 1; f < len; f++) {
+            const uint32_t *x = canon + (size_t)r[e] * 8, *y = canon + (size_t)r[f] * 8;
+            if (lp_same_above(x, y, shift64) && lp_cmp_words(x, y) > 0) { atomicOr(&a.cscal[c * 16 + 9], LPB_DEEP); return; }
+        }
+    for (uint32_t e = 1; e < len; e++) {
+        const uint32_t v = r[e];
+        const uint32_t* x = canon + (size_t)v * 8;
+        uint32_t f = e;
+        while (f > 0 && lp_cmp_words(canon + (size_t)r[f - 1] * 8, x) > 0) { r[f] = r[f - 1]; f--; }
+        r[f] = v;
+    }
+    for (uint32_t e = 0; e < len; e++) idx[lo + e] = r[e];
+    atomicAdd(&a.cscal[c * 16 + 10], 1u);
 }
 ZK_KERNEL void lpb_tiemask_kernel(LpbArgs a, const uint32_t* idx_sorted) {
     __shared__ uint32_t lor[8];
@@ -199,21 +259,22 @@
     __syncthreads();
     if (threadIdx.x < 8 && lor[threadIdx.x]) atomicOr(&a.cscal[s * 16 + threadIdx.x], lor[threadIdx.x]);
 }
-ZK_KERNEL void lpb_rekey_kernel(LpbArgs a, const uint32_t* fcols, const uint32_t* fshift, const uint32_t* idx_in, uint2* key_out, uint32_t* idx_out) {
-    const uint32_t f = blockIdx.y, i = blockIdx.x * blockDim.x + threadIdx.x;
+ZK_KERNEL void lpb_rekey_kernel(LpbArgs a, LpbBufs b, const LpbRow* rows) {
+    const uint32_t i = blockIdx.x * blockDim.x + threadIdx.x;
     if (i >= a.u) return;
-    const uint32_t c = fcols[f], shift = fshift[f];
-    const uint32_t r = idx_in ? idx_in[(size_t)f * a.u + i] : i;
-    const uint32_t* w = reinterpret_cast<const uint32_t*>(a.canon) + ((size_t)c * a.u + r) * 8;
-    const uint32_t ws = shift >> 5, bs = shift & 31;
+    const LpbRow r = rows[blockIdx.y];
+    const uint32_t row = r.src == LPB_IDENTITY ? i : b.i[r.src][(size_t)r.slot * a.u + i];
+    if (r.out == LPB_SORTED) { b.sorted[(size_t)r.col * a.u + i] = row; return; }
+    const uint32_t* w = reinterpret_cast<const uint32_t*>(a.canon) + ((size_t)r.col * a.u + row) * 8;
+    const uint32_t ws = r.shift >> 5, bs = r.shift & 31;
     uint32_t x[3];
 #pragma unroll
     for (int j = 0; j < 3; j++) x[j] = ws + j < 8 ? w[ws + j] : 0u;
     uint2 k;
     k.x = bs ? (x[0] >> bs) | (x[1] << (32 - bs)) : x[0];
     k.y = bs ? (x[1] >> bs) | (x[2] << (32 - bs)) : x[1];
-    key_out[(size_t)f * a.u + i] = k;
-    idx_out[(size_t)f * a.u + i] = r;
+    b.k[r.out][(size_t)r.slot * a.u + i] = k;
+    b.i[r.out][(size_t)r.slot * a.u + i] = row;
 }
 ZK_KERNEL void lpb_mark_kernel(LpbArgs a, const uint32_t* idx_sorted) {
     const uint32_t l = blockIdx.y, i = blockIdx.x * blockDim.x + threadIdx.x, u = a.u;
@@ -339,10 +400,10 @@
     const uint32_t nwg = (u + FS_TILE - 1) / FS_TILE, nxs = (u + XS_TILE - 1) / XS_TILE + 1;
     size_t off = 0;
     auto take = [&](size_t bytes) { size_t o = off; off += (bytes + 255) & ~(size_t)255; return o; };
-    const size_t o_canon = take((size_t)C * u * 32), o_blind = take((size_t)S * nb * 32), o_ka = take((size_t)C * u * 8), o_kb = take((size_t)C * u * 8),
-                 o_ia = take((size_t)C * u * 4), o_ib = take((size_t)C * u * 4), o_fl = take((size_t)S * u * 4), o_rk = take((size_t)S * u * 4),
+    const size_t o_canon = take((size_t)C * u * 32), o_blind = take((size_t)S * nb * 32),
+                 o_ia = take((size_t)C * u * 4), o_fl = take((size_t)S * u * 4), o_rk = take((size_t)S * u * 4),
                  o_lo = take((size_t)count * u * 4), o_gh = take((size_t)C * nwg * 256 * 4), o_xs = take((size_t)S * nxs * 4), o_sc = take((size_t)count * 64),
-                 o_cs = take((size_t)C * 64), o_sh = take((size_t)C * 4), o_tc = take((size_t)count * 4), o_cp = take((size_t)S * sizeof(void*)),
+                 o_cs = take((size_t)C * 64), o_ca = take((size_t)C * 32), o_sh = take((size_t)C * 4), o_s64 = take((size_t)C * 4), o_ls = take((size_t)C * 4), o_tc = take((size_t)count * 4), o_cp = take((size_t)S * sizeof(void*)),
                  o_op = take((size_t)S * sizeof(void*)), o_sp = take((size_t)C * sizeof(void*));
     ZK_HIP(ctx->ws_tmp.ensure(off + 256));
     char* base = (char*)ctx->ws_tmp.p;
@@ -363,95 +424,133 @@
     ZK_HIP(hipMemcpyAsync(base + o_blind, blind.data(), blind.size(), hipMemcpyHostToDevice, st));
     ZK_HIP(hipMemsetAsync(base + o_sc, 0, count * 64, st));
     ZK_HIP(hipMemsetAsync(base + o_cs, 0, (size_t)C * 64, st));
+    ZK_HIP(hipMemsetAsync(base + o_ca, 0, (size_t)C * 32, st));
     LpbArgs a;
     memset(&a, 0, sizeof a);
     a.cols = (const void* const*)(base + o_cp); a.outs = (void* const*)(base + o_op); a.scols = (const void* const*)(base + o_sp);
     a.tabcol = (const uint32_t*)(base + o_tc);
     a.u = u; a.n = n; a.nb = nb; a.S = S; a.C = C; a.nwg = nwg; a.nxs = nxs;
-    a.canon = base + o_canon; a.key_a = (uint2*)(base + o_ka); a.key_b = (uint2*)(base + o_kb); a.idx_a = (uint32_t*)(base + o_ia); a.idx_b = (uint32_t*)(base + o_ib);
+    a.canon = base + o_canon; a.sorted = (uint32_t*)(base + o_ia);
     a.flags = (uint32_t*)(base + o_fl); a.ranks = (uint32_t*)(base + o_rk); a.leftover = (uint32_t*)(base + o_lo); a.ghist = (uint32_t*)(base + o_gh);
-    a.xsums = (uint32_t*)(base + o_xs); a.scal = (uint32_t*)(base + o_sc); a.cscal = (uint32_t*)(base + o_cs); a.shifts = (const uint32_t*)(base + o_sh);
+    a.xsums = (uint32_t*)(base + o_xs); a.scal = (uint32_t*)(base + o_sc); a.cscal = (uint32_t*)(base + o_cs); a.cnor = (uint32_t*)(base + o_ca); a.shifts = (const uint32_t*)(base + o_sh); a.shifts64 = (const uint32_t*)(base + o_s64);
     a.blind = base + o_blind;
     const int blk = ctx->tune.vec_block;
     const uint32_t g = (u + blk - 1) / blk;
     ZK_LAUNCH(lpb_canon_kernel, dim3(g, C), blk, 0, st, a);
     ZK_CHECK_LAUNCH();
-    std::vector<uint32_t> sc((size_t)count * 16), csc((size_t)C * 16);
+    std::vector<uint32_t> sc((size_t)count * 16), csc((size_t)C * 16), cnor((size_t)C * 8);
     ZK_HIP(hipMemcpyAsync(csc.data(), a.cscal, (size_t)C * 64, hipMemcpyDeviceToHost, st));
+    ZK_HIP(hipMemcpyAsync(cnor.data(), a.cnor, (size_t)C * 32, hipMemcpyDeviceToHost, st));
     ZK_HIP(hipStreamSynchronize(st));
-    std::vector<uint32_t> shifts(C);
-    uint32_t max_bits = 1;
+    uint32_t W = 8;
+    while (W < 64 && (1ull << W) < u) W++;
+    W = std::min(64u, (W + 8 + 7) / 8 * 8);
+    if (ctx->tune.lookup_window_bits > 0) W = (uint32_t)std::min(64, ctx->tune.lookup_window_bits);
+    std::vector<uint32_t> shifts(C), shifts64(C), width(C), width64(C);
     bool any_shift = false;
     for (uint32_t c = 0; c < C; c++) {
         const uint32_t* om = &csc[(size_t)c * 16];
         uint32_t nbits = 1;
         for (int wd = 7; wd >= 0; wd--)
             if (om[wd]) { uint32_t top = 31; while (!((om[wd] >> top) & 1)) top--; nbits = (uint32_t)wd * 32 + top + 1; break; }
-        shifts[c] = nbits > 64 ? nbits - 64 : 0;
+        bool constant = true;
+        for (int wd = 0; wd < 8; wd++) constant &= om[wd] == ~cnor[(size_t)c * 8 + wd];
+        width64[c] = constant ? 0 : std::min(nbits, 64u);
+        width[c] = constant ? 0 : std::min(nbits, W);
+        shifts64[c] = nbits > 64 ? nbits - 64 : 0;
+        shifts[c] = constant ? 0 : nbits - width[c];
         any_shift |= shifts[c] != 0;
-        max_bits = std::max(max_bits, std::min(nbits, 64u));
     }
     ZK_HIP(hipMemcpyAsync(base + o_sh, shifts.data(), (size_t)C * 4, hipMemcpyHostToDevice, st));
-    uint32_t* sorted = a.idx_a;
-    const bool use_order_check = any_shift;
-
-    auto compact_sort = [&](const std::vector<uint32_t>& fcols, const std::vector<std::vector<uint32_t>>& stage_shift, const std::vector<uint32_t>& stage_bits) -> int {
+    ZK_HIP(hipMemcpyAsync(base + o_s64, shifts64.data(), (size_t)C * 4, hipMemcpyHostToDevice, st));
+    uint32_t* sorted = a.sorted;
+    uint32_t* viol = a.ranks;
+
+    std::vector<std::vector<LpbRow>> row_keep;
+    auto compact_sort = [&](const std::vector<uint32_t>& fcols, const std::vector<std::vector<uint32_t>>& stage_shift, const std::vector<std::vector<uint32_t>>& stage_bits) -> int {
         const uint32_t Fn = (uint32_t)fcols.size();
         if (!Fn) return ZK_OK;
+        const size_t T = stage_shift.size();
+        std::vector<LpbRow> rows;
+        struct Launch { uint32_t kind, first, n, pass; };
+        std::vector<Launch> launches;
+        std::vector<uint32_t> cur(Fn, LPB_IDENTITY);
+        for (size_t t = 0; t < T; t++) {
+            const bool last_stage = t + 1 == T;
+            uint32_t max_ps = 0;
+            Launch rk{0, (uint32_t)rows.size(), 0, 0};
+            for (uint32_t f = 0; f < Fn; f++) {
+                const uint32_t ps = (stage_bits[t][f] + 7) / 8;
+                max_ps = std::max(max_ps, ps);
+                if (!ps && !last_stage) continue;
+                const uint32_t out = ps ? (cur[f] == LPB_IDENTITY ? 0u : 1u - cur[f]) : LPB_SORTED;
+                rows.push_back(LpbRow{f, fcols[f], cur[f], out, stage_shift[t][f]});
+                cur[f] = out;
+                rk.n++;
+            }
+            if (rk.n) launches.push_back(rk);
+            for (uint32_t p = 0; p < max_ps; p++) {
+                Launch ln{1, (uint32_t)rows.size(), 0, p};
+                for (uint32_t f = 0; f < Fn; f++) {
+                    const uint32_t ps = (stage_bits[t][f] + 7) / 8;
+                    if (p >= ps) continue;
+                    const uint32_t out = last_stage && p + 1 == ps ? LPB_SORTED : 1u - cur[f];
+                    rows.push_back(LpbRow{f, fcols[f], cur[f], out, 0});
+                    cur[f] = out;
+                    ln.n++;
+                }
+                launches.push_back(ln);
+            }
+        }
         const size_t per = (size_t)Fn * u;
         size_t o2 = 0;
         auto take2 = [&](size_t bytes) { size_t o = o2; o2 += (bytes + 255) & ~(size_t)255; return o; };
         const size_t q_ka = take2(per * 8), q_kb = take2(per * 8), q_ia = take2(per * 4), q_ib = take2(per * 4), q_gh = take2((size_t)Fn * nwg * 256 * 4),
-                     q_fc = take2((size_t)Fn * 4), q_fs = take2((size_t)Fn * 4 * stage_shift.size());
+                     q_rw = take2(rows.size() * sizeof(LpbRow));
         ZK_HIP(ctx->ws_mid.ensure(o2 + 256));
         char* b2 = (char*)ctx->ws_mid.p;
-        uint2 *rk_in = (uint2*)(b2 + q_ka), *rk_out = (uint2*)(b2 + q_kb);
-        uint32_t *ri_in = (uint32_t*)(b2 + q_ia), *ri_out = (uint32_t*)(b2 + q_ib), *rgh = (uint32_t*)(b2 + q_gh);
-        ZK_HIP(hipMemcpyAsync(b2 + q_fc, fcols.data(), (size_t)Fn * 4, hipMemcpyHostToDevice, st));
-        for (size_t t = 0; t < stage_shift.size(); t++)
-            ZK_HIP(hipMemcpyAsync(b2 + q_fs + t * Fn * 4, stage_shift[t].data(), (size_t)Fn * 4, hipMemcpyHostToDevice, st));
-        const uint32_t* order = nullptr;
-        for (size_t t = 0; t < stage_shift.size(); t++) {
-            ZK_LAUNCH(lpb_rekey_kernel, dim3(g, Fn), blk, 0, st, a, (const uint32_t*)(b2 + q_fc), (const uint32_t*)(b2 + q_fs + t * Fn * 4), order, rk_in, ri_in);
+        LpbBufs bufs;
+        bufs.k[0] = (uint2*)(b2 + q_ka); bufs.k[1] = (uint2*)(b2 + q_kb); bufs.i[0] = (uint32_t*)(b2 + q_ia); bufs.i[1] = (uint32_t*)(b2 + q_ib); bufs.sorted = sorted;
+        uint32_t* rgh = (uint32_t*)(b2 + q_gh);
+        const LpbRow* drows = (const LpbRow*)(b2 + q_rw);
+        ZK_HIP(hipMemcpyAsync(b2 + q_rw, rows.data(), rows.size() * sizeof(LpbRow), hipMemcpyHostToDevice, st));
+        for (const Launch& ln : launches) {
+            if (ln.kind == 0) {
+                ZK_LAUNCH(lpb_rekey_kernel, dim3(g, ln.n), blk, 0, st, a, bufs, drows + ln.first);
+                ZK_CHECK_LAUNCH();
+                continue;
+            }
+            ZK_LAUNCH(lpb_hist_kernel, dim3(nwg, ln.n), FS_T, 0, st, bufs, drows + ln.first, u, ln.pass, rgh, nwg);
             ZK_CHECK_LAUNCH();
-            const uint32_t ps = (stage_bits[t] + 7) / 8;
-            for (uint32_t p = 0; p < ps; p++) {
-                ZK_LAUNCH(lpb_hist_kernel, dim3(nwg, Fn), FS_T, 0, st, (const uint2*)rk_in, u, p, rgh, nwg);
-                ZK_CHECK_LAUNCH();
-                ZK_LAUNCH(lpb_offsets_kernel, Fn, 256, 0, st, rgh, nwg);
-                ZK_CHECK_LAUNCH();
-                ZK_LAUNCH(lpb_scatter_kernel, dim3(nwg, Fn), FS_T, 0, st, (const uint2*)rk_in, (const uint32_t*)ri_in, rk_out, ri_out, u, p, (const uint32_t*)rgh, nwg);
-                ZK_CHECK_LAUNCH();
-                std::swap(rk_in, rk_out);
-                std::swap(ri_in, ri_out);
-            }
-            std::swap(rk_in, rk_out);
-            std::swap(ri_in, ri_out);
-            order = ri_out;
-        }
-        for (uint32_t f = 0; f < Fn; f++)
-            ZK_HIP(hipMemcpyAsync(sorted + (size_t)fcols[f] * u, order + (size_t)f * u, (size_t)u * 4, hipMemcpyDeviceToDevice, st));
+            ZK_LAUNCH(lpb_offsets_kernel, ln.n, 256, 0, st, rgh, nwg);
+            ZK_CHECK_LAUNCH();
+            ZK_LAUNCH(lpb_scatter_kernel, dim3(nwg, ln.n), FS_T, 0, st, bufs, drows + ln.first, u, ln.pass, (const uint32_t*)rgh, nwg);
+            ZK_CHECK_LAUNCH();
+            ctx->last_ms["lookup_radix_passes"] += 1.0;
+            ctx->last_ms["lookup_column_passes"] += (double)ln.n;
+        }
+        row_keep.push_back(std::move(rows));
         return ZK_OK;
     };
     auto low_stages = [&](const std::vector<uint32_t>& fcols, const std::vector<uint32_t>& lo_bit, const std::vector<uint32_t>& hi_bit,
-                          std::vector<std::vector<uint32_t>>& stage_shift, std::vector<uint32_t>& stage_bits) {
+                          const std::vector<uint32_t>& win_shift, const std::vector<uint32_t>& win_bits,
+                          std::vector<std::vector<uint32_t>>& stage_shift, std::vector<std::vector<uint32_t>>& stage_bits) {
         const uint32_t Fn = (uint32_t)fcols.size();
         uint32_t n_low = 0;
         for (uint32_t f = 0; f < Fn; f++) if (lo_bit[f] < 256) n_low = std::max(n_low, (hi_bit[f] - lo_bit[f]) / 64 + 1);
         for (uint32_t t = 0; t < n_low; t++) {
-            std::vector<uint32_t> sh(Fn);
-            uint32_t bits = 1;
+            std::vector<uint32_t> sh(Fn, 0), bits(Fn, 0);
             for (uint32_t f = 0; f < Fn; f++) {
                 const uint32_t st_lo = lo_bit[f] == 256 ? 256 : lo_bit[f] + 64 * t;
-                if (st_lo > hi_bit[f] || st_lo >= 256) { sh[f] = 255; continue; }
+                if (st_lo > hi_bit[f] || st_lo >= 256) continue;
                 sh[f] = st_lo;
-                bits = std::max(bits, std::min(64u, hi_bit[f] - st_lo + 1));
+                bits[f] = std::min(64u, hi_bit[f] - st_lo + 1);
             }
             stage_shift.push_back(sh); stage_bits.push_back(bits);
         }
-        std::vector<uint32_t> sh(Fn);
-        for (uint32_t f = 0; f < Fn; f++) sh[f] = shifts[fcols[f]];
-        stage_shift.push_back(sh); stage_bits.push_back(max_bits);
+        std::vector<uint32_t> sh(Fn), bits(Fn);
+        for (uint32_t f = 0; f < Fn; f++) { sh[f] = win_shift[fcols[f]]; bits[f] = win_bits[fcols[f]]; }
+        stage_shift.push_back(sh); stage_bits.push_back(bits);
     };
     auto tie_ranges = [&](const std::vector<uint32_t>& cols_, std::vector<uint32_t>& lo_bit, std::vector<uint32_t>& hi_bit) -> int {
         for (uint32_t c : cols_) ZK_HIP(hipMemsetAsync((char*)a.cscal + (size_t)c * 64, 0, 32, st));
@@ -465,47 +564,90 @@
         }
         return ZK_OK;
     };
+    auto upload_list = [&](const std::vector<uint32_t>& list) -> int {
+        ZK_HIP(hipMemcpyAsync(base + o_ls, list.data(), list.size() * 4, hipMemcpyHostToDevice, st));
+        return ZK_OK;
+    };
 
     const uint64_t hint_key = ((uint64_t)count << 40) ^ ((uint64_t)C << 20) ^ k;
     std::vector<uint32_t>& hint = ctx->lookup_tie_hint[hint_key];
     if (hint.size() != C) hint.assign(C, 0);
-    std::vector<uint32_t> plain, hinted;
-    for (uint32_t c = 0; c < C; c++) (hint[c] && shifts[c] ? hinted : plain).push_back(c);
+    auto sort_columns = [&](const std::vector<uint32_t>& which, const std::vector<uint32_t>& win_shift, const std::vector<uint32_t>& win_bits) -> int {
+        std::vector<uint32_t> plain, hinted;
+        for (uint32_t c : which) (hint[c] && shifts64[c] && win_bits[c] ? hinted : plain).push_back(c);
+        {
+            std::vector<std::vector<uint32_t>> ss(1, std::vector<uint32_t>(plain.size())), sb(1, std::vector<uint32_t>(plain.size()));
+            for (size_t f = 0; f < plain.size(); f++) { ss[0][f] = win_shift[plain[f]]; sb[0][f] = win_bits[plain[f]]; }
+            int rc = compact_sort(plain, ss, sb);
+            if (rc) return rc;
+        }
+        if (!hinted.empty()) {
+            std::vector<uint32_t> lo_bit(hinted.size(), 0), hi_bit(hinted.size());
+            for (size_t f = 0; f < hinted.size(); f++) hi_bit[f] = std::min(shifts64[hinted[f]] - 1, hint[hinted[f]] - 1 + 16);
+            std::vector<std::vector<uint32_t>> ss, sb;
+            low_stages(hinted, lo_bit, hi_bit, win_shift, win_bits, ss, sb);
+            int rc = compact_sort(hinted, ss, sb);
+            if (rc) return rc;
+        }
+        return ZK_OK;
+    };
+    std::vector<uint32_t> all(C);
+    for (uint32_t c = 0; c < C; c++) all[c] = c;
+    for (uint32_t c = 0; c < C; c++) if (hint[c] && shifts64[c]) ctx->last_ms["lookup_hinted_sorts"] += 1.0;
     {
-        std::vector<std::vector<uint32_t>> ss(1, std::vector<uint32_t>(plain.size()));
-        for (size_t f = 0; f < plain.size(); f++) ss[0][f] = shifts[plain[f]];
-        int rc = compact_sort(plain, ss, {max_bits});
+        int rc = sort_columns(all, shifts, width);
         if (rc) return rc;
     }
-    if (!hinted.empty()) {
-        std::vector<uint32_t> lo_bit(hinted.size(), 0), hi_bit(hinted.size());
-        for (size_t f = 0; f < hinted.size(); f++) hi_bit[f] = std::min(shifts[hinted[f]] - 1, hint[hinted[f]] - 1 + 16);
-        std::vector<std::vector<uint32_t>> ss; std::vector<uint32_t> sb;
-        low_stages(hinted, lo_bit, hi_bit, ss, sb);
-        int rc = compact_sort(hinted, ss, sb);
-        if (rc) return rc;
-        ctx->last_ms["lookup_hinted_sorts"] += (double)hinted.size();
-    }
-    if (use_order_check) {
-        ZK_LAUNCH(lpb_check_kernel, dim3(g, C), blk, 0, st, a, (const uint32_t*)sorted); ZK_CHECK_LAUNCH();
+    if (any_shift) {
+        ZK_LAUNCH(lpb_check_kernel, dim3(g, C), blk, 0, st, a, (const uint32_t*)sorted, (const uint32_t*)nullptr, viol); ZK_CHECK_LAUNCH();
         ZK_HIP(hipMemcpyAsync(csc.data(), a.cscal, (size_t)C * 64, hipMemcpyDeviceToHost, st));
         ZK_HIP(hipStreamSynchronize(st));
-        std::vector<uint32_t> fcols;
-        for (uint32_t c = 0; c < C; c++) if (csc[(size_t)c * 16 + 8]) fcols.push_back(c);
-        if (!fcols.empty()) {
-            std::vector<uint32_t> lo_bit, hi_bit;
-            int rc = tie_ranges(fcols, lo_bit, hi_bit);
+        std::vector<uint32_t> tied, recheck, full;
+        for (uint32_t c = 0; c < C; c++) if (csc[(size_t)c * 16 + 8]) tied.push_back(c);
+        if (!tied.empty()) {
+            int rc = upload_list(tied);
             if (rc) return rc;
-            std::vector<std::vector<uint32_t>> ss; std::vector<uint32_t> sb;
-            low_stages(fcols, lo_bit, hi_bit, ss, sb);
-            rc = compact_sort(fcols, ss, sb);
+            ZK_LAUNCH(lpb_repair_kernel, dim3(g, (uint32_t)tied.size()), blk, 0, st, a, (const uint32_t*)(base + o_ls), sorted, (const uint32_t*)viol); ZK_CHECK_LAUNCH();
+            ZK_HIP(hipMemcpyAsync(csc.data(), a.cscal, (size_t)C * 64, hipMemcpyDeviceToHost, st));
+            ZK_HIP(hipStreamSynchronize(st));
+            for (uint32_t c : tied) {
+                (csc[(size_t)c * 16 + 9] ? full : recheck).push_back(c);
+                ZK_HIP(hipMemsetAsync((char*)a.cscal + (size_t)c * 64 + 32, 0, 4, st));
+            }
+            ctx->last_ms["lookup_repaired_sorts"] += (double)recheck.size();
+        }
+        if (!full.empty()) {
+            for (uint32_t c : full) shifts[c] = shifts64[c];
+            ZK_HIP(hipMemcpyAsync(base + o_sh, shifts.data(), (size_t)C * 4, hipMemcpyHostToDevice, st));
+            int rc = sort_columns(full, shifts64, width64);
             if (rc) return rc;
-            for (size_t f = 0; f < fcols.size(); f++) {
-                hint[fcols[f]] = hi_bit[f] + 1;
-                ZK_HIP(hipMemsetAsync((char*)a.cscal + (size_t)fcols[f] * 64 + 32, 0, 4, st));
+            rc = upload_list(full);
+            if (rc) return rc;
+            ZK_LAUNCH(lpb_check_kernel, dim3(g, (uint32_t)full.size()), blk, 0, st, a, (const uint32_t*)sorted, (const uint32_t*)(base + o_ls), (uint32_t*)nullptr); ZK_CHECK_LAUNCH();
+            ZK_HIP(hipMemcpyAsync(csc.data(), a.cscal, (size_t)C * 64, hipMemcpyDeviceToHost, st));
+            ZK_HIP(hipStreamSynchronize(st));
+            std::vector<uint32_t> fcols;
+            for (uint32_t c : full) if (csc[(size_t)c * 16 + 8]) fcols.push_back(c);
+            if (!fcols.empty()) {
+                std::vector<uint32_t> lo_bit, hi_bit;
+                rc = tie_ranges(fcols, lo_bit, hi_bit);
+                if (rc) return rc;
+                std::vector<std::vector<uint32_t>> ss, sb;
+                low_stages(fcols, lo_bit, hi_bit, shifts64, width64, ss, sb);
+                rc = compact_sort(fcols, ss, sb);
+                if (rc) return rc;
+                for (size_t f = 0; f < fcols.size(); f++) {
+                    hint[fcols[f]] = hi_bit[f] + 1;
+                    ZK_HIP(hipMemsetAsync((char*)a.cscal + (size_t)fcols[f] * 64 + 32, 0, 4, st));
+                    recheck.push_back(fcols[f]);
+                }
+                ctx->last_ms["lookup_refined_sorts"] += (double)fcols.size();
             }
-            ZK_LAUNCH(lpb_check_kernel, dim3(g, C), blk, 0, st, a, (const uint32_t*)sorted); ZK_CHECK_LAUNCH();
-            ctx->last_ms["lookup_refined_sorts"] += (double)fcols.size();
+        }
+        if (!recheck.empty()) {
+            int rc = upload_list(recheck);
+            if (rc) return rc;
+            ZK_LAUNCH(lpb_check_kernel, dim3(g, (uint32_t)recheck.size()), blk, 0, st, a, (const uint32_t*)sorted, (const uint32_t*)(base + o_ls), (uint32_t*)nullptr); ZK_CHECK_LAUNCH();
         }
     }
     ZK_LAUNCH(lpb_fill_unconsumed_kernel, dim3(g, (uint32_t)count), blk, 0, st, a);
```

New measurement: 73320. About the same (-0.1%).
